# EPFL-VILAB/MultiMAE

Hardware: AMD Instinct MI355X
Metric: pre-train images/sec (whole node), ViT-B RGB+D+S 224^2 98-vis-tok (higher is better)
Workload: dtype bf16 (fp32_output_adapters: fp16 storage); 1 GPU; BASELINE.json configs[2]: ViT-B, RGB+depth+semseg, 224^2, Dirichlet alpha=1.0, 98 visible tokens, 4 cross-attention decoders (dim 256, depth 2), semseg adapter (fp32_output_adapters) with fp16 STORAGE (activations / saved tensors / gradients of the adapter as IEEE half in HBM: every matmul input carries the 11-bit significand TF32 gave the reference on A100; gradients stored times a power of two f; per_gpu_batch=256, global_batch=256, parallelism=dp1

## Files before the change

include/mmae.h:

```cpp
#ifndef MMAE_H
#define MMAE_H

#include <stddef.h>
#include <stdint.h>

#ifdef __cplusplus
extern "C" {
#endif

#define MMAE_ABI_VERSION 7

#define MMAE_F32  0
#define MMAE_BF16 1
#define MMAE_F32X3 2
#define MMAE_F32F16 3
#define MMAE_MXFP8 4

#define MMAE_F16 5

#define MMAE_EINVAL   (-1)
#define MMAE_ELAUNCH  (-2)
#define MMAE_ESUPPORT (-3)

int mmae_abi_version(void);
int mmae_struct_size(int which);
const char* mmae_last_error(void);

#define MMAE_EPI_NONE  0
#define MMAE_EPI_GELU  1
#define MMAE_EPI_DGELU 2
#define MMAE_EPI_GELU_G 3
#define MMAE_EPI_MUL   4

typedef struct mmae_gemm_desc {
    const void* A; const void* B; void* C;
    int32_t ab_dtype;
    int32_t c_dtype;
    int32_t M, N, K;
    int32_t a_trans, b_trans;
    int64_t lda, ldb, ldc;
    int32_t batch, batch_inner;
    int64_t sA_outer, sA_inner, sB_outer, sB_inner, sC_outer, sC_inner;
    const float* bias;
    const float* resid;
    int64_t ldr;
    void* aux;
    int64_t ldaux;
    int32_t aux_dtype;
    int32_t epi;
    int32_t accumulate;
    float alpha;
    int32_t tile;
    int32_t split_k;
    void* ws;
    int64_t ws_elems;
    float* colsum_part;
    float* a_colsum;
    int32_t a_colsum_acc;
    const void* a_scale;
    const void* b_scale;
    void* q_out; void* q_scale;
    int64_t ldq;
    const float* a_amax;
    const float* ln_gamma; const float* ln_beta; void* ln_out; float* ln_mean; float* ln_rstd; float ln_eps;
} mmae_gemm_desc;

int mmae_gemm(const mmae_gemm_desc* d, void* stream);
int mmae_gemm_plan(const mmae_gemm_desc* d, int* tile, int* split_k);
int mmae_gemm_auto_splitk(int M, int N, int K, int ab_dtype);
int mmae_gemm_cu_reserve(int k);
int mmae_gemm_cu_share(int k);
int mmae_gemm_side_cus(int k);
#ifdef MMAE_EXPERIMENTS
int mmae_gemm_duo_occupancy(int tile);
#endif

int64_t mmae_mx_scale_bytes(int rows, int cols);
int mmae_mx_quant(const void* x, int x_dtype, int64_t ldx, int rows, int cols, void* q, int64_t ldq, void* scales, void* stream);
int mmae_mx_quant_t(const void* w, int w_dtype, int64_t ldw, int n, int k, void* q, int64_t ldq, void* scales, void* stream);
int mmae_mx_quant_rows_t(const void* x, int x_dtype, int64_t ldx, int M, int C, void* q, int64_t ldq, void* scales, void* stream);
int mmae_mx_wgrad(int on);
int mmae_gelu_grad_aux(int on);
int mmae_ln_fuse(int on);
int mmae_xattn_fuse(int on);
int mmae_mx_scale_clear(void* scales, int rows, int cols, void* stream);
int mmae_layernorm_fwd_mx(const float* x, const float* gamma, const float* beta, void* y_bf16, float* mean, float* rstd, int64_t R, int D,
                          float eps, void* q, void* scales, void* stream);
int mmae_attn_fwd_mx(const void* q, const void* k, const void* v, void* o, float* lse, int B, int H, int Nq, int Nk, int hd,
                     int64_t q_sb, int64_t q_sr, int64_t k_sb, int64_t k_sr, int64_t v_sb, int64_t v_sr, int64_t o_sb, int64_t o_sr,
                     float scale, void* mx_q, void* mx_scale, void* stream);
int mmae_attn_bwd_mx(const void* q, const void* k, const void* v, const void* o, const void* d_o, const float* lse, void* dq, void* dk,
                     void* dv, int B, int H, int Nq, int Nk, int hd, int64_t q_sb, int64_t q_sr, int64_t k_sb, int64_t k_sr, int64_t v_sb,
                     int64_t v_sr, int64_t o_sb, int64_t o_sr, int64_t dq_sb, int64_t dq_sr, int64_t dk_sb, int64_t dk_sr, int64_t dv_sb,
                     int64_t dv_sr, float scale, void* mx_q, void* mx_scale, void* stream);
int64_t mmae_mx_tmp_bytes(int rows, int cols);
int mmae_mx_prepare_weights(int n, const void* const* w, int w_dtype, const int32_t* n_out, const int32_t* k_in, void* const* dst, void* stream);
int mmae_probe_mx_mfma(const int32_t* a_64x8, const int32_t* b_64x8, const int32_t* scale_a_64, const int32_t* scale_b_64, int opsel_a, int opsel_b,
                       float* out_64x16, void* stream);

int mmae_gemm_timing_enable(int on);
int mmae_gemm_timing_read(double* ms3, double* flop3, int64_t* calls3);
int mmae_gemm_timing_read_bytes(double* bytes3);

typedef struct mmae_dw_problem {
    const void* dy; int64_t ldy;
    const void* x; int64_t ldx;
    float* dw; float* db;
    int32_t n_out, k_in;
} mmae_dw_problem;

typedef struct mmae_dw_group_desc {
    int32_t n, rows, ab_dtype, accumulate, split_k;
    mmae_dw_problem p[8];
    float* ws; int64_t ws_elems;
    const float* unscale;
} mmae_dw_group_desc;

int64_t mmae_gemm_dw_group_ws_elems(const mmae_dw_group_desc* d);
int mmae_gemm_dw_group(const mmae_dw_group_desc* d, void* stream);

int mmae_layernorm_fwd(const float* x, const float* gamma, const float* beta, void* y, int y_dtype,
                       float* mean, float* rstd, int64_t R, int D, float eps, void* stream);
int mmae_layernorm_bwd_nblk(int64_t R);
int mmae_layernorm_bwd(const void* dy, int dy_dtype, const float* x, const float* gamma,
                       const float* mean, const float* rstd, const float* dx_in, float* dx_out,
                       void* dx_act, int dx_act_dtype, float* part, int64_t R, int D, void* stream);
int mmae_colsum_partials(const float* part, float* out, int nrows, int ncols, int accumulate, void* stream);

int64_t mmae_colsum_ws_elems(int64_t M, int N);
int mmae_colsum(const void* dy, int dtype, int64_t M, int N, int64_t ld, float* out, int accumulate,
                float* ws, void* stream);
int mmae_colsum_scatter(const void* dy, int dtype, int64_t M, int N, int64_t ld, int seg_w, const void* dsts_host,
                        int nseg, int accumulate, float* ws, void* stream);

#define MMAE_COLSUM_MAX_JOBS 8
typedef struct mmae_colsum_job {
    const void* src; int32_t dtype; int32_t cols; int64_t rows; int64_t ld;
    int32_t seg_w; int32_t nseg; float* dst[8];
    const float* unscale;
} mmae_colsum_job;
int64_t mmae_colsum_batch_ws_elems(const mmae_colsum_job* jobs, int n);
int mmae_colsum_batch(const mmae_colsum_job* jobs, int n, int accumulate, float* ws, int64_t ws_elems, void* stream);

int mmae_softmax_fwd(const float* S, int64_t lds_, void* P, int p_dtype, int64_t ldp, int64_t rows, int n,
                     float scale, void* stream);
int mmae_softmax_bwd(const void* P, int p_dtype, int64_t ldp, const float* dP, int64_t lddp, void* dS,
                     int64_t ldds, int64_t rows, int n, float scale, void* stream);

int mmae_xattn_fwd_fused(const void* qn, const void* cn, const void* wq, const float* bq, const void* wkv, const float* bkv, void* q, void* kv,
                         void* out, float* lse, int B, int H, int Nq, int Nk, int D, float scale, void* stream);
int mmae_attn_fwd(const void* q, const void* k, const void* v, void* o, float* lse, int B, int H, int Nq, int Nk, int hd,
                  int64_t q_sb, int64_t q_sr, int64_t k_sb, int64_t k_sr, int64_t v_sb, int64_t v_sr, int64_t o_sb,
                  int64_t o_sr, float scale, void* stream);
int mmae_attn_bwd(const void* q, const void* k, const void* v, const void* o, const void* d_o, const float* lse, void* dq,
                  void* dk, void* dv, int B, int H, int Nq, int Nk, int hd, int64_t q_sb, int64_t q_sr, int64_t k_sb,
                  int64_t k_sr, int64_t v_sb, int64_t v_sr, int64_t o_sb, int64_t o_sr, int64_t dq_sb, int64_t dq_sr,
                  int64_t dk_sb, int64_t dk_sr, int64_t dv_sb, int64_t dv_sr, float scale, void* stream);
int mmae_attn_fwd_f32x3(const void* q, const void* k, const void* v, void* o, float* lse, int B, int H, int Nq, int Nk, int hd,
                  int64_t q_sb, int64_t q_sr, int64_t k_sb, int64_t k_sr, int64_t v_sb, int64_t v_sr, int64_t o_sb,
                  int64_t o_sr, float scale, void* stream);
int mmae_attn_bwd_f32x3(const void* q, const void* k, const void* v, const void* o, const void* d_o, const float* lse, void* dq,
                  void* dk, void* dv, int B, int H, int Nq, int Nk, int hd, int64_t q_sb, int64_t q_sr, int64_t k_sb,
                  int64_t k_sr, int64_t v_sb, int64_t v_sr, int64_t o_sb, int64_t o_sr, int64_t dq_sb, int64_t dq_sr,
                  int64_t dk_sb, int64_t dk_sr, int64_t dv_sb, int64_t dv_sr, float scale, void* stream);
int mmae_attn_fwd_f32f16(const void* q, const void* k, const void* v, void* o, float* lse, int B, int H, int Nq, int Nk, int hd,
                  int64_t q_sb, int64_t q_sr, int64_t k_sb, int64_t k_sr, int64_t v_sb, int64_t v_sr, int64_t o_sb,
// ... 310 lines not shown
```

multimae_amd/_lib.py:

```python
from __future__ import annotations

import ctypes
import os
import re
from typing import Dict, List, Tuple

_PKG = os.path.dirname(os.path.abspath(__file__))
HEADER = os.path.join(os.path.dirname(_PKG), 'include', 'mmae.h')
LIB_PATH = os.environ.get('MMAE_LIB') or os.path.join(_PKG, 'libmmae_hip.so')

F32, BF16, F32X3, F32F16 = 0, 1, 2, 3
MXFP8 = 4
F16 = 5
U16, I32 = 6, 7
EPI_NONE, EPI_GELU, EPI_DGELU, EPI_GELU_G, EPI_MUL = 0, 1, 2, 3, 4


class GemmDesc(ctypes.Structure):
    _fields_ = [
        ('A', ctypes.c_void_p), ('B', ctypes.c_void_p), ('C', ctypes.c_void_p),
        ('ab_dtype', ctypes.c_int32), ('c_dtype', ctypes.c_int32),
        ('M', ctypes.c_int32), ('N', ctypes.c_int32), ('K', ctypes.c_int32),
        ('a_trans', ctypes.c_int32), ('b_trans', ctypes.c_int32),
        ('lda', ctypes.c_int64), ('ldb', ctypes.c_int64), ('ldc', ctypes.c_int64),
# ... 71 lines not shown


class OptGroupsDesc(ctypes.Structure):
    _fields_ = [('p', _P), ('g', _P), ('m', _P), ('v', _P), ('n', _L), ('shadow', _P), ('shadow_dtype', _I),
                ('beta1', _F), ('beta2', _F), ('eps', _F), ('clip_grad', _F), ('skip_grad', _F), ('grad_prescale', _F),
                ('loss_dev', _P), ('state', _P), ('istate', _P), ('ws', _P), ('found_inf_dev', _P), ('grad_scale_dev', _P),
                ('group_map', _P), ('n_groups', _I), ('hyper', _P), ('hyper_dev', _P)]


OPT_MAX_GROUPS = 256


class PatchSrc(ctypes.Structure):
    _fields_ = [
        ('data', ctypes.c_void_p), ('emb', ctypes.c_void_p),
        ('kind', ctypes.c_int32), ('C', ctypes.c_int32), ('H', ctypes.c_int32), ('W', ctypes.c_int32),
        ('ph', ctypes.c_int32), ('pw', ctypes.c_int32), ('k_off', ctypes.c_int32), ('n_cls', ctypes.c_int32),
    ]


_SCALARS = {
    'int': ctypes.c_int, 'int32_t': ctypes.c_int32, 'int64_t': ctypes.c_int64, 'float': ctypes.c_float,
    'size_t': ctypes.c_size_t,
}
_RET = {'int': ctypes.c_int, 'int64_t': ctypes.c_int64, 'const char*': ctypes.c_char_p}


def _parse_header(path: str) -> Dict[str, Tuple[object, List[object]]]:
    src = open(path).read()
    if not os.environ.get('MMAE_EXPERIMENTS'):
        src = re.sub(r'#ifdef\s+MMAE_EXPERIMENTS.*?#endif', ' ', src, flags=re.S)
    src = re.sub(r'/\*.*?\*/', ' ', src, flags=re.S)
    src = re.sub(r'//[^\n]*', ' ', src)
    src = re.sub(r'typedef\s+struct\s+\w+\s*\{.*?\}\s*\w+\s*;', ' ', src, flags=re.S)
    protos = {}
    for m in re.finditer(r'(const\s+char\s*\*|int64_t|int)\s+(mmae_\w+)\s*\(([^)]*)\)\s*;', src):
        ret = re.sub(r'\s+', ' ', m.group(1)).replace(' *', '*')
        name, args = m.group(2), m.group(3).strip()
        argtypes = []
        if args and args != 'void':
            for a in args.split(','):
                a = a.strip()
                if '*' in a:
                    argtypes.append(ctypes.c_void_p)
                else:
                    ty = a.split()[-2] if len(a.split()) >= 2 else a
                    argtypes.append(_SCALARS[ty])
        protos[name] = (_RET[ret], argtypes)
    return protos


_PROTOS = _parse_header(HEADER) if os.path.exists(HEADER) else {}
_lib = None


def declared_symbols() -> List[str]:
    return sorted(_PROTOS)


def load() -> ctypes.CDLL:
    global _lib
    if _lib is not None:
        return _lib
    if not os.path.exists(LIB_PATH):
        raise RuntimeError(
            f'{LIB_PATH} not found: the MI355X kernel library is not built. '
            'Run `python -c "import __graft_entry__ as g; g.build()"` (or `make -C multimae_amd/csrc`). '
            'multimae_amd has no CPU / PyTorch fallback by design.')
    lib = ctypes.CDLL(LIB_PATH)
    for name, (ret, argtypes) in _PROTOS.items():
        fn = getattr(lib, name)
        fn.restype = ret
        fn.argtypes = argtypes
    if lib.mmae_abi_version() != 7:
        raise RuntimeError('libmmae_hip.so ABI version mismatch')
    for which, cls in enumerate((GemmDesc, BlockDesc, StackDesc, AdapterDesc, OptDesc, PatchSrc, DwGroupDesc, ColsumJob,
                                     OptGroupsDesc)):
        if lib.mmae_struct_size(which) != ctypes.sizeof(cls):
            raise RuntimeError(f'{cls.__name__}: ctypes mirror ({ctypes.sizeof(cls)} B) != library struct ({lib.mmae_struct_size(which)} B)')
    if os.environ.get('MMAE_MX_WGRAD') is not None:
        lib.mmae_mx_wgrad(int(os.environ['MMAE_MX_WGRAD'] != '0'))
    if os.environ.get('MMAE_LN_FUSE') is not None:
        lib.mmae_ln_fuse(int(os.environ['MMAE_LN_FUSE'] != '0'))
    if os.environ.get('MMAE_XATTN_FUSE') is not None:
        lib.mmae_xattn_fuse(int(os.environ['MMAE_XATTN_FUSE'] != '0'))
    if os.environ.get('MMAE_GELU_GRAD_AUX') is not None:
        lib.mmae_gelu_grad_aux(int(os.environ['MMAE_GELU_GRAD_AUX'] != '0'))
    _lib = lib
    return lib


class KernelError(RuntimeError):
    pass


def check(rc: int, what: str) -> None:
    if rc != 0:
        msg = load().mmae_last_error()
        raise KernelError(f'{what} failed (rc={rc}): {msg.decode() if msg else "?"}')
```

multimae_amd/csrc/common.h:

```cpp
#pragma once
#include <hip/hip_runtime.h>
#include <stdint.h>
#include <atomic>
#include "../../include/mmae.h"

typedef __attribute__((ext_vector_type(8))) __bf16 bf16x8;
typedef __attribute__((ext_vector_type(4))) short s16x4;
typedef __attribute__((ext_vector_type(4))) int i32x4;
typedef __attribute__((ext_vector_type(2))) int i32x2;
typedef __attribute__((ext_vector_type(16))) float f32x16;
typedef __attribute__((ext_vector_type(4))) float f32x4;
typedef __attribute__((ext_vector_type(2))) float f32x2;

#define MMAE_WAVE 64

void mmae_set_error(const char* msg);
int mmae_check_launch(const char* what);
int mmae_cu_count();
int mmae_cu_side();
int mmae_cu_avail();
int mmae_depth_standardize_int(const void* x, int x_dtype, float* y, int B, int n, int lo, int hi, float eps, hipStream_t stream);

#include <stdlib.h>
static inline int mmae_env_int(const char* name, int dflt) {
// ... 98 lines not shown
    o[2] = f16_bits_to_f32((uint16_t)((uint32_t)r[1] & 0xffffu)); o[3] = f16_bits_to_f32((uint16_t)((uint32_t)r[1] >> 16));
    return o;
}
__device__ __forceinline__ void st4(h16_t* p, f32x4 v) {
    i32x2 r;
    r[0] = (int)((uint32_t)f32_to_f16_bits(v[0]) | ((uint32_t)f32_to_f16_bits(v[1]) << 16));
    r[1] = (int)((uint32_t)f32_to_f16_bits(v[2]) | ((uint32_t)f32_to_f16_bits(v[3]) << 16));
    *reinterpret_cast<i32x2*>(p) = r;
}

__device__ __forceinline__ void gelu_cdf_exp(float x, float& cdf, float& e) {
    const float z = fabsf(x) * 0.70710678118654752f;
    const float t = __builtin_amdgcn_rcpf(1.0f + 0.3275911f * z);
    float p = 1.061405429f;
    p = p * t - 1.453152027f; p = p * t + 1.421413741f; p = p * t - 0.284496736f; p = p * t + 0.254829592f;
    e = __expf(-z * z);
    const float h = 0.5f * p * t * e;
    cdf = x < 0.f ? h : 1.0f - h;
}
__device__ __forceinline__ float gelu_erf(float x) { float c, e; gelu_cdf_exp(x, c, e); return x * c; }
__device__ __forceinline__ void gelu_both(float x, float& y, float& dy) { float c, e; gelu_cdf_exp(x, c, e); y = x * c; dy = c + x * e * 0.39894228040143268f; }
__device__ __forceinline__ float gelu_erf_grad(float x) { float c, e; gelu_cdf_exp(x, c, e); return c + x * e * 0.39894228040143268f; }

__device__ __forceinline__ void gelu_both_fast2(f32x2 x, f32x2& y, f32x2& dy) {
    f32x2 t;
    t[0] = __builtin_amdgcn_fmed3f(x[0], -4.0f, 4.0f);
    t[1] = __builtin_amdgcn_fmed3f(x[1], -4.0f, 4.0f);
    const f32x2 s = t * t;
    f32x2 q = {8.063375031e-11f, 8.063375031e-11f}, r = {9.796052989e-10f, 9.796052989e-10f};
#define MMAE_PK_STEP(acc, c) acc = __builtin_elementwise_fma(acc, s, (f32x2){c, c})
    MMAE_PK_STEP(q, -7.003438364e-09f); MMAE_PK_STEP(r, -8.218800834e-08f);
    MMAE_PK_STEP(q, 2.716148569e-07f);  MMAE_PK_STEP(r, 3.028347546e-06f);
    MMAE_PK_STEP(q, -6.294988571e-06f); MMAE_PK_STEP(r, -6.495757385e-05f);
    MMAE_PK_STEP(q, 9.890799001e-05f);  MMAE_PK_STEP(r, 9.073266031e-04f);
    MMAE_PK_STEP(q, -1.133921717e-03f); MMAE_PK_STEP(r, -8.716320413e-03f);
    MMAE_PK_STEP(q, 9.877475989e-03f);  MMAE_PK_STEP(r, 5.845610030e-02f);
    MMAE_PK_STEP(q, -6.641059427e-02f); MMAE_PK_STEP(r, -2.648265329e-01f);
    MMAE_PK_STEP(q, 3.989227094e-01f);  MMAE_PK_STEP(r, 7.976095497e-01f);
#undef MMAE_PK_STEP
    const f32x2 half = {0.5f, 0.5f};
    const f32x2 cdf = __builtin_elementwise_fma(t, q, half);
    f32x2 xm;
    xm[0] = __builtin_amdgcn_fmed3f(x[0], -4.0f, 3.402823466e38f);
    xm[1] = __builtin_amdgcn_fmed3f(x[1], -4.0f, 3.402823466e38f);
    y = __builtin_elementwise_fma(xm, cdf, x * (f32x2){0.f, 0.f});
    dy = __builtin_elementwise_fma(t, r, half);
}
__device__ __forceinline__ void gelu_both_fast4(f32x4 x, f32x4& y, f32x4& dy) {
    f32x2 ya, da, yb, db;
    gelu_both_fast2((f32x2){x[0], x[1]}, ya, da);
    gelu_both_fast2((f32x2){x[2], x[3]}, yb, db);
    y = (f32x4){ya[0], ya[1], yb[0], yb[1]};
    dy = (f32x4){da[0], da[1], db[0], db[1]};
}
__device__ __forceinline__ f32x4 gelu_grad_fast4(f32x4 x) { f32x4 y, dy; gelu_both_fast4(x, y, dy); return dy; }

__device__ __forceinline__ int mx_shared_exp(float amax) {
    const unsigned b = __float_as_uint(amax);
    const int e = (int)((b >> 23) & 0xffu) - 8 + ((b & 0x7fffffu) > 0x600000u ? 1 : 0);
    return e < 0 ? 0 : e;
}
__device__ __forceinline__ float mx_inv_scale(int e) { return __uint_as_float((unsigned)(254 - e) << 23); }
__device__ __forceinline__ float mx_clamp448(float v) { return __builtin_amdgcn_fmed3f(v, -448.0f, 448.0f); }
__device__ __forceinline__ int mx_cvt4_e4m3(float a, float b, float c, float d) {
    int r = 0;
    r = __builtin_amdgcn_cvt_pk_fp8_f32(mx_clamp448(a), mx_clamp448(b), r, false);
    r = __builtin_amdgcn_cvt_pk_fp8_f32(mx_clamp448(c), mx_clamp448(d), r, true);
    return r;
}
__device__ __forceinline__ long long mx_scale_addr(long long rows, long long r, int kb) {
    return (((long long)(kb >> 3) * rows + r) * 2 + (kb & 1)) * 4 + ((kb >> 1) & 3);
}

__device__ __forceinline__ float wave_sum(float v) {
#pragma unroll
    for (int o = 32; o > 0; o >>= 1) v += __shfl_xor(v, o, 64);
    return v;
}
__device__ __forceinline__ float wave_max(float v) {
#pragma unroll
    for (int o = 32; o > 0; o >>= 1) v = fmaxf(v, __shfl_xor(v, o, 64));
    return v;
}
__device__ __forceinline__ float join4_sum(const float* sh) { return ((sh[0] + sh[1]) + sh[2]) + sh[3]; }
__device__ __forceinline__ float join4_max(const float* sh) { return fmaxf(fmaxf(sh[0], sh[1]), fmaxf(sh[2], sh[3])); }
template <class T, class Op>
__device__ __forceinline__ T block_tree(T v, T* s, Op op) {
    s[threadIdx.x] = v;
    __syncthreads();
    for (int o = 128; o > 0; o >>= 1) {
        if ((int)threadIdx.x < o) s[threadIdx.x] = op(s[threadIdx.x], s[threadIdx.x + o]);
        __syncthreads();
    }
    return s[0];
}
__device__ __forceinline__ double block_tree_sum(double v, double* s) {
    return block_tree(v, s, [](double a, double b) { return a + b; });
}
__device__ __forceinline__ float block_tree_max(float v, float* s) {
    return block_tree(v, s, [](float a, float b) { return fmaxf(a, b); });
}

__device__ __forceinline__ float resize_tap4(float ly0, float ly1, float lx0, float lx1, float a, float b, float c, float d, bool odd) {
#pragma clang fp contract(off)
    const float bot = __builtin_fmaf(lx0, c, lx1 * d);
    if (odd) {
        const float top = __builtin_fmaf(lx1, b, lx0 * a);
        return __builtin_fmaf(ly0, top, ly1 * bot);
    }
    const float top = __builtin_fmaf(lx0, a, lx1 * b);
    return __builtin_fmaf(ly1, bot, ly0 * top);
}

static inline int64_t cdiv64(int64_t a, int64_t b) { return (a + b - 1) / b; }
```

multimae_amd/csrc/composite.hip:

```cpp
#include <math.h>
#include <stdlib.h>
#include <atomic>
#include <mutex>
#include "gemm_common.h"

namespace {

struct Ctx {
    int act_dtype, f32_gemm, grad_acc;
    float* ws_main; int64_t ws_main_elems;
    float* ws_side; int64_t ws_side_elems;
    void* mx_tmp = nullptr; int64_t mx_tmp_bytes = 0;
    const void* const* x3_w = nullptr; int x3_n = 0;
    void* x3_tmp = nullptr; int64_t x3_tmp_bytes = 0;
    const float* dy_amax = nullptr;
    bool b16() const { return act_dtype != MMAE_F32; }
    bool h16() const { return act_dtype == MMAE_F16; }
    int ab() const { return b16() ? act_dtype : f32_gemm; }
    int ab_grad() const { return b16() ? act_dtype : ((f32_gemm == MMAE_F32F16 && !dy_amax) ? MMAE_F32X3 : f32_gemm); }
    const float* amax_for(int ab) const { return ab == MMAE_F32F16 ? dy_amax : nullptr; }
    const float* unscale() const { return h16() ? dy_amax : nullptr; }
    size_t es() const { return b16() ? 2 : 4; }
};
inline bool is16(int act) { return act != MMAE_F32; }
// ... 72 lines not shown
int lin_fwd(const Ctx& c, const void* x, const void* w, const float* bias, void* out, int out_dtype, int M, int N, int K,
            const float* resid, void* aux, int epi, hipStream_t st, const void* const* mxw = nullptr, int mx_in = -1, int mx_out = -1,
            const LnSide* ln = nullptr) {
    mmae_gemm_desc g = {};
    if (ln) { g.ln_gamma = ln->g; g.ln_beta = ln->b; g.ln_out = ln->out; g.ln_mean = ln->mean; g.ln_rstd = ln->rstd; g.ln_eps = ln->eps; }
    g.A = x; g.B = w; g.C = out;
    g.ab_dtype = c.ab();
    g.c_dtype = out_dtype;
    g.M = M; g.N = N; g.K = K;
    g.lda = K; g.ldb = K; g.ldc = N;
    g.batch = g.batch_inner = 1;
    g.bias = bias; g.resid = resid; g.ldr = N;
    g.aux = aux; g.ldaux = N; g.aux_dtype = c.act_dtype;
    g.epi = epi; g.alpha = 1.0f;
    bool x3p = false;
    if (!mxw) {
        int rc3 = 0;
        const void* a3 = nullptr;
        const void* const* t3 = x3_operand(c, x, K, w, M, K, &a3, st, &rc3);
        if (rc3) return rc3;
        if (t3) { g.A = a3; g.B = t3[1]; g.K = 3 * K; g.lda = g.ldb = 3LL * K; g.ab_dtype = MMAE_BF16; x3p = true; }
    }
    if (mxw) {
        int rc = mx_in_operand(c, x, K, M, K, mx_in, mx_out, &g.A, &g.a_scale, st);
        if (rc) return rc;
        if (mx_out >= 0) { if ((rc = mx_slot(c, mx_out, M, N, &g.q_out, &g.q_scale))) return rc; g.ldq = N; }
        g.B = mxw[0]; g.b_scale = mxw[1]; g.ab_dtype = MMAE_MXFP8; g.split_k = 1;
        return mmae_gemm(&g, st);
    }
    int tile = 0, split = 1;
    int rc = mmae_gemm_plan(&g, &tile, &split);
    if (rc) return rc;
    g.tile = tile; g.split_k = split;
    if (split > 1) {
        if ((int64_t)split * M * N > c.ws_main_elems) { mmae_set_error("composite: ws_main too small"); return MMAE_EINVAL; }
        g.ws = c.ws_main; g.ws_elems = c.ws_main_elems;
    }
    return x3p ? mmae_gemm_ex(&g, st, 1, 1.0 / 3.0) : mmae_gemm(&g, st);
}

int lin_dx(const Ctx& c, const void* dy, int64_t ldy, const void* w, void* out, int out_dtype, int M, int N, int K, void* aux, int epi,
           float* colsum_part, hipStream_t st, const void* const* mxw = nullptr, int mx_in = -1, int mx_out = -1) {
    mmae_gemm_desc g = {};
    g.A = dy; g.B = w; g.C = out;
    g.ab_dtype = c.ab_grad(); g.a_amax = c.amax_for(g.ab_dtype);
    if (c.h16() && out_dtype == MMAE_F32) g.a_amax = c.unscale();
    g.c_dtype = out_dtype;
    g.M = M; g.N = K; g.K = N;
    g.lda = ldy; g.ldb = K; g.ldc = K;
    g.b_trans = 1;
    g.batch = g.batch_inner = 1;
    g.aux = aux; g.ldaux = K; g.aux_dtype = c.act_dtype;
    g.epi = epi; g.alpha = 1.0f;
    g.colsum_part = colsum_part;
    bool x3p = false;
    if (!mxw) {
        int rc3 = 0;
        const void* a3 = nullptr;
        const void* const* t3 = x3_operand(c, dy, ldy, w, M, N, &a3, st, &rc3);
        if (rc3) return rc3;
        if (t3) { g.A = a3; g.lda = 3LL * N; g.B = t3[2]; g.K = 3 * N; g.ab_dtype = MMAE_BF16; x3p = true; }
    }
    if (mxw) {
        int rc = mx_in_operand(c, dy, ldy, M, N, mx_in, mx_out, &g.A, &g.a_scale, st);
        if (rc) return rc;
        if (mx_out >= 0) { if ((rc = mx_slot(c, mx_out, M, K, &g.q_out, &g.q_scale))) return rc; g.ldq = K; }
        g.lda = N; g.B = mxw[2]; g.b_scale = mxw[3]; g.ldb = N; g.b_trans = 0; g.ab_dtype = MMAE_MXFP8; g.split_k = 1;
        return mmae_gemm(&g, st);
    }
    int tile = 0, split = 1;
    int rc = mmae_gemm_plan(&g, &tile, &split);
    if (rc) return rc;
    g.tile = tile; g.split_k = split;
    if (split > 1) {
        if ((int64_t)split * M * K > c.ws_main_elems) { mmae_set_error("composite: ws_main too small"); return MMAE_EINVAL; }
        g.ws = c.ws_main; g.ws_elems = c.ws_main_elems;
    }
    return x3p ? mmae_gemm_ex(&g, st, 1, 1.0 / 3.0) : mmae_gemm(&g, st);
}

std::atomic<int> g_gelu_grad_aux{1};
inline int epi_gelu(int act) { return (is16(act) && g_gelu_grad_aux.load(std::memory_order_relaxed)) ? MMAE_EPI_GELU_G : MMAE_EPI_GELU; }
inline int epi_dgelu(int act) { return (is16(act) && g_gelu_grad_aux.load(std::memory_order_relaxed)) ? MMAE_EPI_MUL : MMAE_EPI_DGELU; }

struct ColBatch {
    mmae_colsum_job j[MMAE_COLSUM_MAX_JOBS];
    int n = 0;
    int add(const Ctx& c, const void* src, int dtype, int64_t rows, int cols, int64_t ld, int seg_w, float* const* dsts, int nseg, hipStream_t st) {
        bool any = false;
        for (int i = 0; i < nseg; ++i) any = any || dsts[i];
        if (!any) return 0;
        if (n == MMAE_COLSUM_MAX_JOBS) { const int rc = flush(c, st); if (rc) return rc; }
        mmae_colsum_job& q = j[n++];
        q = mmae_colsum_job{};
        q.src = src; q.dtype = dtype; q.rows = rows; q.cols = cols; q.ld = ld; q.seg_w = seg_w; q.nseg = nseg;
        q.unscale = c.unscale();
        for (int i = 0; i < nseg; ++i) q.dst[i] = dsts[i];
        return 0;
    }
    int add3(const Ctx& c, const float* part, int rows, int seg_w, float* d0, float* d1, float* d2, hipStream_t st) {
        float* dsts[3] = {d0, d1, d2};
        return add(c, part, MMAE_F32, rows, 3 * seg_w, 3 * seg_w, seg_w, dsts, 3, st);
    }
    int add1(const Ctx& c, const void* src, int dtype, int64_t rows, int cols, int64_t ld, float* dst, hipStream_t st) {
        float* dsts[1] = {dst};
        return add(c, src, dtype, rows, cols, ld, cols, dsts, 1, st);
    }
    int flush(const Ctx& c, hipStream_t st) {
        if (n == 0) return 0;
        const int64_t need = mmae_colsum_batch_ws_elems(j, n);
        if (need > c.ws_side_elems) { mmae_set_error("composite: ws_side too small for the batched column sums"); return MMAE_EINVAL; }
        const int rc = mmae_colsum_batch(j, n, c.grad_acc, c.ws_side, c.ws_side_elems, st);
        n = 0;
        return rc;
    }
};

int lin_dw(const Ctx& c, const void* dy, int64_t ldy, const void* x, float* dw, float* db, int M, int N, int K, hipStream_t st, ColBatch* cb = nullptr) {
    if (!dw && !db) return 0;
    const int acc = c.grad_acc;
    if (c.h16() && (dw || !cb)) { mmae_set_error("composite: an fp16-storage weight gradient outside the grouped launch (widths must be multiples of 8)"); return MMAE_ESUPPORT; }
    if (dw) {
        mmae_gemm_desc g = {};
        g.A = dy; g.B = x; g.C = dw;
        g.ab_dtype = c.ab_grad(); g.a_amax = c.amax_for(g.ab_dtype);
        g.c_dtype = MMAE_F32;
        g.M = N; g.N = K; g.K = M;
        g.lda = ldy; g.ldb = K; g.ldc = K;
        g.a_trans = g.b_trans = 1;
        g.batch = g.batch_inner = 1;
        g.accumulate = acc; g.alpha = 1.0f;
        int tile = 0, split = 1;
        int rc = mmae_gemm_plan(&g, &tile, &split);
        if (rc) return rc;
        g.tile = tile; g.split_k = split;
        const bool fused_db = db && tile == 9 && g.ab_dtype == MMAE_BF16;
        const int64_t ws_used = (split > 1 ? (int64_t)split * N * K : 0) + (fused_db ? (int64_t)(split > 1 ? split : 1) * N : 0);
        if (ws_used > c.ws_side_elems) { mmae_set_error("composite: ws_side too small"); return MMAE_EINVAL; }
        if (ws_used) { g.ws = c.ws_side; g.ws_elems = c.ws_side_elems; }
        if (fused_db) { g.a_colsum = db; g.a_colsum_acc = acc; db = nullptr; }
        rc = mmae_gemm(&g, st);
        if (rc) return rc;
    }
    if (db) {
        if (cb) return cb->add1(c, dy, c.act_dtype, M, N, ldy, db, st);
        if (mmae_colsum_ws_elems(M, N) > c.ws_side_elems) { mmae_set_error("composite: ws_side too small"); return MMAE_EINVAL; }
        return mmae_colsum(dy, c.act_dtype, M, N, ldy, db, acc, c.ws_side, st);
    }
    return 0;
}

bool dw_group_enabled() {
    static const bool on = (mmae_env_int("MMAE_DW_GROUP", 1) != 0);
    return on;
}
struct DwGroup {
    mmae_dw_group_desc g;
    bool on;
    int64_t scratch = 0;
    DwGroup(const Ctx& c, int rows) : g{}, on(c.b16() && (dw_group_enabled() || c.h16())) {
        g.rows = rows; g.ab_dtype = c.act_dtype; g.accumulate = c.grad_acc; g.unscale = c.unscale();
    }
    bool add(const void* dy, int64_t ldy, const void* x, int64_t ldx, float* dw, float* db, int n_out, int k_in) {
        if (!on || (!dw && !db) || g.n >= 8 || (n_out % 8) || (k_in % 8) || (ldy % 8) || (ldx % 8)) return false;
        mmae_dw_problem& q = g.p[g.n++];
        q.dy = dy; q.ldy = ldy; q.x = x; q.ldx = ldx; q.dw = dw; q.db = db; q.n_out = n_out; q.k_in = k_in;
// ... 174 lines not shown
    b.n1_w = p[0]; b.n1_b = p[1]; b.qkv_b = p[2]; b.proj_b = p[3]; b.n2_w = p[4]; b.n2_b = p[5]; b.fc1_b = p[6]; b.fc2_b = p[7];
}
void fill_block_act(mmae_block_desc& b, const float* x0, const BlockAct& a) {
    b.x0 = x0; b.ln1 = a.ln1; b.mean1 = a.mean1; b.rstd1 = a.rstd1; b.qkv = a.qkv; b.lse = a.lse; b.ao = a.ao; b.x1 = a.x1;
    b.ln2 = a.ln2; b.mean2 = a.mean2; b.rstd2 = a.rstd2; b.hpre = a.hpre; b.hact = a.hact; b.x2 = a.x2;
}
void fill_block_tmp(mmae_block_desc& b, const BlockTmp& t) {
    b.d_hpre = t.d_hpre; b.d_ln2 = t.d_ln2; b.d_ao = t.d_ao; b.d_qkv = t.d_qkv; b.d_ln1 = t.d_ln1; b.dx1 = t.dx1; b.dx1_act = t.dx1_act;
    b.dx0 = t.dx0; b.dx0_act = t.dx0_act; b.part_h = t.part_h; b.part1 = t.part1; b.part2 = t.part2; b.dxs_act = t.dxs_act;
}
void fill_block_grads(mmae_block_desc& b, float* const* g) {
    b.g_n1_w = g[0]; b.g_n1_b = g[1]; b.g_qkv_w = g[2]; b.g_qkv_b = g[3]; b.g_proj_w = g[4]; b.g_proj_b = g[5];
    b.g_n2_w = g[6]; b.g_n2_b = g[7]; b.g_fc1_w = g[8]; b.g_fc1_b = g[9]; b.g_fc2_w = g[10]; b.g_fc2_b = g[11];
}

struct StackRun {
    int B, N, D, heads, Hd, act, f32g, grad_acc;
    const void* const* w; const float* const* p; const float* const* dp; float* const* g;
    const float* x_in; const BlockAct* acts; BlockTmp* tmps; int nset;
    float* ws_main; int64_t ws_main_elems; float* ws_side; int64_t ws_side_elems;
    const void* const* mx_w = nullptr; void* mx_tmp = nullptr; int64_t mx_tmp_bytes = 0;
    const void* const* x3_w = nullptr; int x3_n = 0; void* x3_tmp = nullptr; int64_t x3_tmp_bytes = 0;
    const float* dy_amax = nullptr;
};

int run_blocks_bwd(const StackRun& s, int lo, int hi, const float* dx_top, const void* dx_top_act, bool top_in_sets, bool first_fc2_b_done,
                   const float* const* extra, float* cs_first, float* dx_final, hipStream_t st, hipStream_t sd,
                   const float** dx_out, const void** dx_out_act) {
    const int64_t R = (int64_t)s.B * s.N;
    const float* dx = dx_top;
    const void* dx_act = dx_top_act;
    bool fc2_done = first_fc2_b_done;
    hipEvent_t side_done[MAX_SETS] = {};
    int rc;
    MMAE_REQUIRE(s.nset >= 1 && s.nset <= MAX_SETS, "stack_bwd: more temporary sets than side-stream progress marks");
    for (int l = hi - 1; l >= lo; --l) {
        BlockTmp t = s.tmps[l % s.nset];
        if (sd != st && l + s.nset < hi + (top_in_sets ? 1 : 0) && side_done[(l + s.nset - 1) % s.nset]) {
            if (hipStreamWaitEvent(st, side_done[(l + s.nset - 1) % s.nset], 0) != hipSuccess) { mmae_set_error("stack_bwd: stream wait failed"); return MMAE_ELAUNCH; }
        }
        if (extra && l < hi - 1 && extra[l]) {
            if ((rc = mmae_axpy_f32((float*)dx, extra[l], 1.0f, R * s.D, st))) return rc;
            if ((rc = cast_to_act(s.act, dx, (void*)dx_act, R * s.D, st))) return rc;
            fc2_done = false;
        }
        mmae_block_desc b = {};
        fill_block_params(b, s.B, s.N, s.D, s.heads, s.Hd, s.act, s.f32g, 0.f, s.w + 4 * l, s.p + 8 * l);
        fill_block_act(b, l == 0 ? s.x_in : s.acts[l - 1].x2, s.acts[l]);
        if (l == lo && dx_final) { t.dx0 = dx_final; }
        fill_block_tmp(b, t);
        b.dx = dx; b.dx_act = dx_act;
        float* none[12] = {};
        fill_block_grads(b, s.g ? s.g + 12 * l : none);
        b.dp1 = s.dp ? s.dp[2 * l] : nullptr; b.dp2 = s.dp ? s.dp[2 * l + 1] : nullptr;
        const bool below_clean = l > 0 && !(extra && extra[l - 1]) && !(s.dp && s.dp[2 * (l - 1) + 1]);
        b.g_cs = l > 0 ? ((below_clean && s.g) ? s.g[12 * (l - 1) + 11] : nullptr) : cs_first;
        b.grad_acc = s.grad_acc; b.fc2_b_done = fc2_done ? 1 : 0;
        b.ws_main = s.ws_main; b.ws_main_elems = s.ws_main_elems; b.ws_side = s.ws_side; b.ws_side_elems = s.ws_side_elems;
        if (s.mx_w) { b.mx_w = s.mx_w + 16 * l; b.mx_tmp = s.mx_tmp; b.mx_tmp_bytes = s.mx_tmp_bytes; }
        b.x3_w = s.x3_w; b.x3_n = s.x3_n; b.x3_tmp = s.x3_tmp; b.x3_tmp_bytes = s.x3_tmp_bytes;
        b.dy_amax = s.dy_amax;
        if ((rc = mmae_block_bwd(&b, st, sd))) return rc;
        if (sd != st) {
            hipEvent_t e = g_held_ring.next();
            if (!e || hipEventRecord(e, sd) != hipSuccess) { mmae_set_error("stack_bwd: event record failed"); return MMAE_ELAUNCH; }
            side_done[l % s.nset] = e;
        }
        fc2_done = b.g_cs != nullptr;
        dx = t.dx0;
        dx_act = is16(s.act) ? (const void*)t.dx0_act : (const void*)t.dx0;
    }
    *dx_out = dx; *dx_out_act = dx_act;
    return 0;
}

}

int mmae_decoder_build_rows(const float* ctx, const int64_t* ids_keep, const int64_t* ids_restore, const float* mask_token,
                            const float* const* task_emb_rows, const float* pos, const int32_t* task_offsets_host, int T, int q_task, int B,
                            int n_keep, int G, int D, int n_q, float* queries, float* context, void* stream);
int mmae_decoder_build_rows_ln(const float* ctx, const int64_t* ids_keep, const int64_t* ids_restore, const float* mask_token,
                               const float* const* task_emb_rows, const float* pos, const int32_t* task_offsets_host, int T, int q_task, int B,
                               int n_keep, int G, int D, int n_q, float* queries, float* context, const BuildLn* ln, int ln_dtype, void* stream);

extern "C" {

static int block_fwd_impl(const mmae_block_desc* d, void* stream, bool ln1_done, const LnSide* next);
int mmae_block_fwd(const mmae_block_desc* d, void* stream) { return block_fwd_impl(d, stream, false, nullptr); }

static int block_fwd_impl(const mmae_block_desc* d, void* stream, bool ln1_done, const LnSide* next) {
    int rc = check_desc(d);
    if (rc) return rc;
    MMAE_REQUIRE(d->x2, "block_fwd: null output");
    MMAE_REQUIRE(!(d->dp1 || d->dp2) || d->branch, "block_fwd: stochastic depth needs the branch scratch buffer");
    hipStream_t st = (hipStream_t)stream;
    const Ctx c = ctx_of(d);
    const int R = d->B * d->N, D = d->D, Hd = d->Hd, act = d->act_dtype;
    const void* const* mx = (d->mx_w && act == MMAE_BF16) ? d->mx_w : nullptr;
    static const bool mx_fuse = (mmae_env_int("MMAE_MX_FUSE", 1) != 0);
    const int pre = (mx && mx_fuse) ? 0 : -1;
    auto ln = [&](const float* x, const float* w, const float* b, void* y, float* mu, float* rs) -> int {
        if (pre < 0) return mmae_layernorm_fwd(x, w, b, y, act, mu, rs, R, D, d->eps, st);
        void *q, *s;
        const int r0 = mx_slot(c, 0, R, D, &q, &s);
        return r0 ? r0 : mmae_layernorm_fwd_mx(x, w, b, y, mu, rs, R, D, d->eps, q, s, st);
    };
    if (!ln1_done && (rc = ln(d->x0, d->n1_w, d->n1_b, d->ln1, d->mean1, d->rstd1))) return rc;
    if ((rc = lin_fwd(c, d->ln1, d->qkv_w, d->qkv_b, d->qkv, act, R, 3 * D, D, nullptr, nullptr, MMAE_EPI_NONE, st, mx, pre))) return rc;
    const bool side = !mx && !d->dp1 && !d->dp2 && ln_side_ok(c, D, D, MMAE_F32) && (Hd % 32) == 0;
    const LnSide ln2s = {d->n2_w, d->n2_b, d->ln2, d->mean2, d->rstd2, d->eps};
    if (pre >= 0) {
        void *aq, *as;
        if ((rc = mx_slot(c, 0, R, D, &aq, &as)) || (rc = attn_strides_fwd(d, st, aq, as))) return rc;
    } else if ((rc = attn_strides_fwd(d, st))) return rc;
    if (d->dp1) {
        if ((rc = lin_fwd(c, d->ao, d->proj_w, d->proj_b, d->branch, MMAE_F32, R, D, D, nullptr, nullptr, MMAE_EPI_NONE, st, mx ? mx + 4 : nullptr, pre))) return rc;
        if ((rc = mmae_rowscale_add(d->x0, d->branch, d->dp1, d->x1, R, d->N, D, st))) return rc;
    } else {
        if ((rc = lin_fwd(c, d->ao, d->proj_w, d->proj_b, d->x1, MMAE_F32, R, D, D, d->x0, nullptr, MMAE_EPI_NONE, st, mx ? mx + 4 : nullptr, pre, -1,
                          side ? &ln2s : nullptr))) return rc;
    }
    if (!side && (rc = ln(d->x1, d->n2_w, d->n2_b, d->ln2, d->mean2, d->rstd2))) return rc;
    const int hq = pre < 0 ? -1 : 1;
    if ((rc = lin_fwd(c, d->ln2, d->fc1_w, d->fc1_b, d->hact, act, R, Hd, D, nullptr, d->hpre, epi_gelu(act), st, mx ? mx + 8 : nullptr, pre, hq))) return rc;
    if (d->dp2) {
        if ((rc = lin_fwd(c, d->hact, d->fc2_w, d->fc2_b, d->branch, MMAE_F32, R, D, Hd, nullptr, nullptr, MMAE_EPI_NONE, st, mx ? mx + 12 : nullptr, hq))) return rc;
        return mmae_rowscale_add(d->x1, d->branch, d->dp2, d->x2, R, d->N, D, st);
    }
    return lin_fwd(c, d->hact, d->fc2_w, d->fc2_b, d->x2, MMAE_F32, R, D, Hd, d->x1, nullptr, MMAE_EPI_NONE, st, mx ? mx + 12 : nullptr, hq, -1,
                   (side && next) ? next : nullptr);
}

static bool block_side_ok(const mmae_block_desc& b) {
    const Ctx c = ctx_of(&b);
    return !(b.mx_w && b.act_dtype == MMAE_BF16) && !b.dp1 && !b.dp2 && ln_side_ok(c, b.D, b.D, MMAE_F32) && (b.Hd % 32) == 0;
}

std::atomic<int> g_xattn_fuse{0};
int mmae_xattn_fuse(int on) {
    const int prev = g_xattn_fuse.load(std::memory_order_relaxed);
    if (on >= 0) g_xattn_fuse.store(on ? 1 : 0, std::memory_order_relaxed);
    return prev;
}

int mmae_ln_fuse(int on) {
    const int prev = g_ln_fuse.load(std::memory_order_relaxed);
    if (on >= 0) g_ln_fuse.store(on ? 1 : 0, std::memory_order_relaxed);
    return prev;
}

int mmae_gelu_grad_aux(int on) {
    const int prev = g_gelu_grad_aux.load(std::memory_order_relaxed);
    if (on >= 0) g_gelu_grad_aux.store(on ? 1 : 0, std::memory_order_relaxed);
    return prev;
}

int mmae_mx_wgrad(int on) {
    const int prev = g_mx_wgrad.load(std::memory_order_relaxed);
    if (on >= 0) g_mx_wgrad.store(on ? 1 : 0, std::memory_order_relaxed);
    return prev;
}

int mmae_block_bwd(const mmae_block_desc* d, void* stream, void* side_stream) {
    int rc = check_desc(d);
    if (rc) return rc;
    MMAE_REQUIRE(d->dx && d->dx_act && d->dx0 && d->d_hpre && d->d_ln2 && d->d_ao && d->d_qkv && d->d_ln1 && d->dx1 && d->part1 && d->part2,
                 "block_bwd: null gradient / temporary buffer");
    const int act = d->act_dtype;
    MMAE_REQUIRE(act == MMAE_F32 || (d->dx1_act && d->dx0_act), "block_bwd: 16-bit activations need dx1_act / dx0_act");
    MMAE_REQUIRE(act != MMAE_F16 || d->dy_amax, "block_bwd: fp16 storage needs dy_amax (the scale its gradients are stored in)");
    MMAE_REQUIRE(!d->g_fc1_b || d->part_h, "block_bwd: part_h needed for the fc1 bias gradient");
    MMAE_REQUIRE(!(d->dp1 || d->dp2) || d->dxs_act, "block_bwd: stochastic depth needs the dxs_act scratch buffer");
    MMAE_REQUIRE(!(d->dp2 && d->fc2_b_done), "block_bwd: with a scaled MLP branch the fc2 bias gradient cannot come from the producer of dx");
    hipStream_t st = (hipStream_t)stream;
    hipStream_t sd = side_stream ? (hipStream_t)side_stream : st;
    const Ctx c = ctx_of(d);
    const int R = d->B * d->N, D = d->D, Hd = d->Hd, N = d->N, hd = D / d->heads;
    const int nblk = mmae_layernorm_bwd_nblk(R);
    const int hrows = (R + 31) / 32;
    const void* dm_act = d->dx_act;
    if (d->dp2) {
        if ((rc = mmae_rowscale_cast(d->dx, d->dp2, d->dxs_act, act, R, N, D, st))) return rc;
        dm_act = d->dxs_act;
    }
    float* part_h = d->g_fc1_b ? d->part_h : nullptr;
    const void* const* mx = (d->mx_w && act == MMAE_BF16) ? d->mx_w : nullptr;
    DwGroup grp(c, R);
    if (d->dp1 || d->dp2) grp.on = false;
    ColBatch cbat;
    ColBatch* const cb_defer = (d->dp1 || d->dp2) ? nullptr : &cbat;
    auto wgrad = [&](const void* dy, int64_t ldy, const void* x, int64_t ldx, float* dw, float* db, int n_out, int k_in) -> int {
        int r = 0;
        if (mx && mx_lin_dw(c, dy, ldy, x, ldx, dw, R, n_out, k_in, sd, &r)) {
            if (r || !db) return r;
            if (mmae_colsum_ws_elems(R, n_out) > c.ws_side_elems) { mmae_set_error("composite: ws_side too small"); return MMAE_EINVAL; }
            return mmae_colsum(dy, c.act_dtype, R, n_out, ldy, db, c.grad_acc, c.ws_side, sd);
        }
        if (grp.add(dy, ldy, x, ldx, dw, db, n_out, k_in)) return 0;
        return lin_dw(c, dy, ldy, x, dw, db, R, n_out, k_in, sd, cb_defer);
    };
    static const bool mx_fuse = (mmae_env_int("MMAE_MX_FUSE", 1) != 0);
    const int hq = (mx && mx_fuse) ? 1 : -1;
    if ((rc = lin_dx(c, dm_act, D, d->fc2_w, d->d_hpre, act, R, D, Hd, d->hpre, epi_dgelu(act), part_h, st, mx ? mx + 12 : nullptr, -1, hq))) return rc;
    if ((rc = fork_to(st, sd))) return rc;
    if ((rc = wgrad(dm_act, D, d->hact, Hd, d->g_fc2_w, d->fc2_b_done ? nullptr : d->g_fc2_b, D, Hd))) return rc;
    if ((rc = lin_dx(c, d->d_hpre, Hd, d->fc1_w, d->d_ln2, act, R, Hd, D, nullptr, MMAE_EPI_NONE, nullptr, st, mx ? mx + 8 : nullptr, hq))) return rc;
    if ((rc = wgrad(d->d_hpre, Hd, d->ln2, D, d->g_fc1_w, nullptr, Hd, D))) return rc;
    if (part_h && (rc = cbat.add1(c, part_h, MMAE_F32, hrows, Hd, Hd, d->g_fc1_b, sd))) return rc;
    void* dx1_act = act == MMAE_F32 ? nullptr : d->dx1_act;
    if ((rc = mmae_layernorm_bwd(d->d_ln2, act, d->x1, d->n2_w, d->mean2, d->rstd2, d->dx, d->dx1, dx1_act, act, d->part2, R, D, st))) return rc;
    const void* da_act = act == MMAE_F32 ? (const void*)d->dx1 : (const void*)d->dx1_act;
    if (d->dp1) {
        if (d->dp2 && (rc = fork_to(sd, st))) return rc;
        if ((rc = mmae_rowscale_cast(d->dx1, d->dp1, d->dxs_act, act, R, N, D, st))) return rc;
        da_act = d->dxs_act;
    }
    if ((rc = lin_dx(c, da_act, D, d->proj_w, d->d_ao, act, R, D, D, nullptr, MMAE_EPI_NONE, nullptr, st, mx ? mx + 4 : nullptr))) return rc;
    if ((rc = fork_to(st, sd))) return rc;
    if ((rc = cbat.add3(c, d->part2, nblk, D, d->g_n2_w, d->g_n2_b, d->dp1 ? nullptr : d->g_proj_b, sd))) return rc;
    if ((rc = wgrad(da_act, D, d->ao, D, d->g_proj_w, d->dp1 ? d->g_proj_b : nullptr, D, D))) return rc;
    {
        const size_t es = es_of(act);
        const char* qkv = (const char*)d->qkv;
        char* dq = (char*)d->d_qkv;
        const int64_t sb3 = (int64_t)N * 3 * D, sb1 = (int64_t)N * D;
        auto fn = act == MMAE_BF16 ? mmae_attn_bwd : (act == MMAE_F16 ? mmae_attn_bwd_f16 : mmae_attn_bwd_f32x3);
        if (act == MMAE_F32 && c.ab_grad() == MMAE_F32F16) {
            if ((rc = mmae_attn_bwd_f32f16(qkv, qkv + (size_t)D * es, qkv + (size_t)2 * D * es, d->ao, d->d_ao, d->lse, dq, dq + (size_t)D * es,
                                           dq + (size_t)2 * D * es, d->B, d->heads, N, N, hd, sb3, 3 * D, sb3, 3 * D, sb3, 3 * D, sb1, D, sb3, 3 * D,
                                           sb3, 3 * D, sb3, 3 * D, 1.0f / sqrtf((float)hd), c.dy_amax, st))) return rc;
        } else if (N > 256) {
            const int64_t nd = (int64_t)d->B * d->heads * N;
            MMAE_REQUIRE(d->ws_main && d->ws_main_elems >= nd, "block_bwd: ws_main too small for the attention delta (B * heads * N f32)");
            if ((rc = mmae_attn_bwd_tiled(qkv, qkv + (size_t)D * es, qkv + (size_t)2 * D * es, d->ao, d->d_ao, d->lse, d->ws_main, dq, dq + (size_t)D * es,
                                          dq + (size_t)2 * D * es, d->B, d->heads, N, N, hd, sb3, 3 * D, sb3, 3 * D, sb3, 3 * D, sb1, D, sb3, 3 * D, sb3, 3 * D,
                                          sb3, 3 * D, 1.0f / sqrtf((float)hd), st))) return rc;
// ... 83 lines not shown
    MMAE_REQUIRE(d->tmp && d->tmp_bytes >= mmae_stack_tmp_bytes(d) && d->act_bytes >= mmae_stack_act_bytes(d), "stack_bwd: slab too small");
    MMAE_REQUIRE(0 <= d->l_begin && d->l_begin < d->l_end && d->l_end <= d->L, "stack_bwd: bad block range");
    MMAE_REQUIRE(d->d_out && d->d_out[d->L - 1], "stack_bwd: the gradient of the last block's output is required");
    MMAE_REQUIRE(d->l_begin > 0 || d->dx, "stack_bwd: null dx");
    hipStream_t st = (hipStream_t)stream;
    hipStream_t sd = side_stream ? (hipStream_t)side_stream : st;
    const size_t es = d->act_dtype == MMAE_BF16 ? 2 : 4;
    const bool bf = d->act_dtype == MMAE_BF16;
    const int64_t RD = (int64_t)d->B * d->N * d->D;
    Carver ca(d->act);
    BlockAct acts[64];
    for (int l = 0; l < d->L; ++l) acts[l] = carve_block_act(ca, d->B, d->N, d->D, d->heads, d->Hd, es);
    Carver ct(d->tmp);
    const int nset = d->L < NSET ? d->L : NSET;
    BlockTmp tmps[NSET];
    for (int s = 0; s < nset; ++s) tmps[s] = carve_block_tmp(ct, d->B, d->N, d->D, d->Hd, es, bf, stack_has_dp(d));
    void* top_act = bf ? ct.take(RD * es) : nullptr;
    void* mx_tmp = d->mx_w ? ct.take(stack_mx_tmp_bytes(d)) : nullptr;
    if (d->l_end < d->L && (rc = fork_to(sd, st))) return rc;
    const float* dx; const void* dx_act;
    bool fc2_done = false;
    if (d->l_end == d->L) {
        dx = d->d_out[d->L - 1];
        if (bf) { if ((rc = mmae_cast_f32_to_bf16(dx, top_act, RD, st))) return rc; dx_act = top_act; } else dx_act = dx;
    } else {
        const BlockTmp& t = tmps[d->l_end % nset];
        dx = t.dx0; dx_act = bf ? (const void*)t.dx0_act : (const void*)t.dx0;
        const int le = d->l_end;
        const bool clean = !(d->d_out[le - 1]) && !(d->dp && d->dp[2 * (le - 1) + 1]);
        fc2_done = clean && d->g && d->g[12 * (le - 1) + 11];
        if (d->d_out[le - 1]) {
            if ((rc = mmae_axpy_f32((float*)dx, d->d_out[le - 1], 1.0f, RD, st))) return rc;
            if (bf && (rc = mmae_cast_f32_to_bf16(dx, (void*)dx_act, RD, st))) return rc;
        }
    }
    StackRun s = {d->B, d->N, d->D, d->heads, d->Hd, d->act_dtype, d->f32_gemm, d->grad_acc, d->w, d->p, d->dp, d->g, d->x, acts, tmps, nset,
                  d->ws_main, d->ws_main_elems, d->ws_side, d->ws_side_elems};
    if (d->mx_w) { s.mx_w = d->mx_w; s.mx_tmp = mx_tmp; s.mx_tmp_bytes = stack_mx_tmp_bytes(d); }
    const float* o; const void* oa;
    return run_blocks_bwd(s, d->l_begin, d->l_end, dx, dx_act, d->l_end < d->L, fc2_done, d->d_out, nullptr, d->l_begin == 0 ? d->dx : nullptr, st, sd, &o, &oa);
}

namespace {

struct AdapterAct {
    float *ctx_tok, *te, *queries, *context, *qmean, *qrstd, *cmean, *crstd, *lse, *x, *omean, *orstd, *x1, *pat;
    void *enc_act, *qn, *cn, *q, *kv, *xo, *on, *hpre, *hact, *h_act;
    BlockAct blocks[MAX_SETS];
    void* x3_tmp;
};
int kp_of(const mmae_adapter_desc* d) { return d->C * d->ph * d->pw; }
int64_t adapter_x3_bytes(const mmae_adapter_desc* d) {
    if (!d->x3_w || d->act_dtype != MMAE_F32) return 0;
    int wide = d->Hd > 3 * d->D ? d->Hd : 3 * d->D;
    if (d->Denc > wide) wide = d->Denc;
    if (kp_of(d) % 32 == 0 && kp_of(d) > wide) wide = kp_of(d);
    const int64_t rq = (int64_t)d->B * d->n_q, rc = (int64_t)d->B * d->NC;
    return mmae_x3_tmp_bytes(rq > rc ? rq : rc, wide);
}

AdapterAct carve_adapter_act(Carver& cv, const mmae_adapter_desc* d) {
    const size_t es = es_of(d->act_dtype);
    const int64_t Rq = (int64_t)d->B * d->n_q, Rc = (int64_t)d->B * d->NC;
    const int D = d->D;
    AdapterAct a;
    a.enc_act = (is16(d->act_dtype) && !d->enc_act) ? cv.take(Rc * d->Denc * es) : nullptr;
    a.ctx_tok = cv.takeT<float>(Rc * D); a.te = cv.takeT<float>((int64_t)d->T * D);
    a.queries = cv.takeT<float>(Rq * D); a.context = cv.takeT<float>(Rc * D);
    a.qn = cv.take(Rq * D * es); a.cn = cv.take(Rc * D * es);
    a.qmean = cv.takeT<float>(Rq); a.qrstd = cv.takeT<float>(Rq); a.cmean = cv.takeT<float>(Rc); a.crstd = cv.takeT<float>(Rc);
    a.q = cv.take(Rq * D * es); a.kv = cv.take(Rc * 2 * D * es); a.xo = cv.take(Rq * D * es);
    a.lse = cv.takeT<float>((int64_t)d->B * d->heads * d->n_q);
    a.x = cv.takeT<float>(Rq * D); a.on = cv.take(Rq * D * es); a.omean = cv.takeT<float>(Rq); a.orstd = cv.takeT<float>(Rq);
    a.hpre = cv.take(Rq * d->Hd * es); a.hact = cv.take(Rq * d->Hd * es); a.x1 = cv.takeT<float>(Rq * D);
    for (int l = 0; l < d->depth; ++l) a.blocks[l] = carve_block_act(cv, d->B, d->n_q, D, d->heads, d->Hd, es);
    a.h_act = is16(d->act_dtype) ? cv.take(Rq * D * es) : nullptr;
    a.pat = d->pat ? d->pat : cv.takeT<float>(Rq * kp_of(d));
    a.x3_tmp = adapter_x3_bytes(d) ? cv.take(adapter_x3_bytes(d)) : nullptr;
    return a;
}

struct AdapterTmp {
    void *d_pat, *dh_act, *d_hpre, *d_on, *dx_act, *d_xo, *d_q, *d_kv, *d_qn, *d_cn, *d_ctx_act;
    float *dh, *part_h, *dx, *part_o, *d_queries, *part_q, *d_context, *part_c, *d_ctx, *part_b;
    BlockTmp blocks[MAX_SETS];
    void* x3_tmp;
};
int64_t ldpat_of(const mmae_adapter_desc* d) { return (kp_of(d) + 7) / 8 * 8; }

AdapterTmp carve_adapter_tmp(Carver& cv, const mmae_adapter_desc* d) {
    const size_t es = es_of(d->act_dtype);
    const bool bf = is16(d->act_dtype);
    const int64_t Rq = (int64_t)d->B * d->n_q, Rc = (int64_t)d->B * d->NC;
    const int D = d->D;
    AdapterTmp t;
    t.d_pat = cv.take(Rq * ldpat_of(d) * es);
    t.dh_act = cv.take(Rq * D * es);
    t.dh = bf ? cv.takeT<float>(Rq * D) : nullptr;
    for (int l = 0; l < d->depth; ++l) t.blocks[l] = carve_block_tmp(cv, d->B, d->n_q, D, d->Hd, es, bf, false);
    t.part_h = cv.takeT<float>((Rq + 31) / 32 * d->Hd);
    t.d_hpre = cv.take(Rq * d->Hd * es); t.d_on = cv.take(Rq * D * es);
    t.dx = cv.takeT<float>(Rq * D); t.dx_act = bf ? cv.take(Rq * D * es) : nullptr;
    t.part_o = cv.takeT<float>((int64_t)mmae_layernorm_bwd_nblk(Rq) * 3 * D);
    t.d_xo = cv.take(Rq * D * es); t.d_q = cv.take(Rq * D * es); t.d_kv = cv.take(Rc * 2 * D * es);
    t.d_qn = cv.take(Rq * D * es); t.d_cn = cv.take(Rc * D * es);
    t.d_queries = cv.takeT<float>(Rq * D); t.part_q = cv.takeT<float>((int64_t)mmae_layernorm_bwd_nblk(Rq) * 3 * D);
    t.d_context = cv.takeT<float>(Rc * D); t.part_c = cv.takeT<float>((int64_t)mmae_layernorm_bwd_nblk(Rc) * 3 * D);
    t.d_ctx = cv.takeT<float>(Rc * D); t.part_b = cv.takeT<float>((int64_t)mmae_decoder_build_bwd_nblk(d->B) * (d->T + 1) * D);
    t.d_ctx_act = bf ? cv.take(Rc * D * es) : nullptr;
    t.x3_tmp = adapter_x3_bytes(d) ? cv.take(adapter_x3_bytes(d)) : nullptr;
    return t;
}

int check_adapter(const mmae_adapter_desc* d) {
    MMAE_REQUIRE(d, "adapter: null descriptor");
    MMAE_REQUIRE(d->B > 0 && d->NC > 0 && d->Denc > 0 && d->D > 0 && d->heads > 0 && d->Hd > 0 && d->D % d->heads == 0 && d->depth >= 0 &&
                 d->depth <= MAX_SETS && d->T >= 1 && d->T <= 7 && d->q_task >= -1 && d->q_task < d->T && d->G >= 0 && d->n_q > 0 && d->NC > d->G,
                 "adapter: bad geometry");
    MMAE_REQUIRE(d->C > 0 && d->nh > 0 && d->nw > 0 && d->ph > 0 && d->pw > 0 && d->nh * d->nw == d->n_q, "adapter: bad patch geometry");
    MMAE_REQUIRE(d->act_dtype == MMAE_BF16 || d->act_dtype == MMAE_F16 || (d->act_dtype == MMAE_F32 && (d->f32_gemm == MMAE_F32X3 || d->f32_gemm == MMAE_F32F16)),
                 "adapter: activations must be bf16, fp16 (MMAE_F16), or f32 with split-bf16 (MMAE_F32X3) / fp16-operand (MMAE_F32F16) products");
    if (d->act_dtype == MMAE_F16 && ((d->D % 32) || (d->Denc % 32) || (d->Hd % 32) || (kp_of(d) % 8))) {
        mmae_set_error("adapter: fp16 storage needs D, Denc, Hd multiples of 32 and C * ph * pw a multiple of 8"); return MMAE_ESUPPORT;
    }
    const int hd = d->D / d->heads;
    if ((hd != 32 && hd != 64) || d->n_q > 256 || d->NC > 256) { mmae_set_error("adapter: geometry outside the fused attention kernel"); return MMAE_ESUPPORT; }
    if (d->act_dtype == MMAE_F32 && mmae_attn_bwd_lds_bytes(1, d->n_q, d->NC, hd) > MMAE_LDS_BYTES) { mmae_set_error("adapter: f32 attention tiles exceed the LDS"); return MMAE_ESUPPORT; }
    if ((d->D % 8) || (d->Denc % 8) || (d->Hd % 8) || (kp_of(d) % 4)) { mmae_set_error("adapter: widths must be multiples of 8 (patch row of 4)"); return MMAE_ESUPPORT; }
    MMAE_REQUIRE(d->task_offsets_host && d->w && d->p && d->mask_token && d->task_emb && d->pos && d->enc && d->ids_keep && d->ids_restore && d->act,
                 "adapter: null pointer");
    MMAE_REQUIRE(is16(d->act_dtype) || d->enc_act == nullptr || d->enc_act == (const void*)d->enc, "adapter: enc_act must alias enc for f32 activations");
    return 0;
}

Ctx ctx_of(const mmae_adapter_desc* d, void* x3_tmp) {
    Ctx c{d->act_dtype, d->f32_gemm, d->grad_acc, d->ws_main, d->ws_main_elems, d->ws_side, d->ws_side_elems};
    if (x3_tmp) { c.x3_w = d->x3_w; c.x3_n = d->x3_n; c.x3_tmp = x3_tmp; c.x3_tmp_bytes = adapter_x3_bytes(d); }
    c.dy_amax = d->dy_amax;
    return c;
}

}

int64_t mmae_adapter_act_bytes(const mmae_adapter_desc* d) {
    if (!d || d->depth < 0 || d->depth > MAX_SETS) return 0;
    Carver cv(nullptr);
    (void)carve_adapter_act(cv, d);
    return cv.off;
}
int64_t mmae_adapter_tmp_bytes(const mmae_adapter_desc* d) {
    if (!d || d->depth < 0 || d->depth > MAX_SETS) return 0;
    Carver cv(nullptr);
    (void)carve_adapter_tmp(cv, d);
    return cv.off;
}
int64_t mmae_adapter_pat_offset(const mmae_adapter_desc* d) {
    if (!d || d->depth < 0 || d->depth > MAX_SETS) return -1;
    Carver cv(nullptr);
    AdapterAct a = carve_adapter_act(cv, d);
    return d->pat ? -1 : (int64_t)(uintptr_t)a.pat;
}

int mmae_adapter_fwd(const mmae_adapter_desc* d, void* stream) {
    int rc = check_adapter(d);
    if (rc) return rc;
    MMAE_REQUIRE(d->act_bytes >= mmae_adapter_act_bytes(d), "adapter_fwd: activation slab too small");
    hipStream_t st = (hipStream_t)stream;
    const int act = d->act_dtype, D = d->D, Hd = d->Hd, B = d->B, NC = d->NC, n_q = d->n_q, T = d->T, depth = d->depth;
    const int Rq = B * n_q, Rc = B * NC, hd = D / d->heads, KP = kp_of(d);
    Carver cv(d->act);
    AdapterAct a = carve_adapter_act(cv, d);
    const Ctx c = ctx_of(d, a.x3_tmp);
    const size_t es = c.es();
    const void* const* w = d->w; const float* const* p = d->p;
    const void *qw = w[0], *kvw = w[1], *pw = w[2], *f1w = w[3], *f2w = w[4], *ow = w[5 + 4 * depth], *pcw = w[6 + 4 * depth];
    const float *qb = p[0], *kvb = p[1], *pb = p[2], *cnw = p[3], *cnb = p[4], *qnw = p[5], *qnb = p[6], *onw = p[7], *onb = p[8], *f1b = p[9],
                *f2b = p[10], *ob = p[11 + 8 * depth], *pcb = p[12 + 8 * depth];
    const void* enc_act = act == MMAE_F32 ? (const void*)d->enc : d->enc_act;
    if (!enc_act) {
        if ((rc = cast_to_act(act, d->enc, a.enc_act, (int64_t)Rc * d->Denc, st))) return rc;
        enc_act = a.enc_act;
    }
    if ((rc = lin_fwd(c, enc_act, pcw, pcb, a.ctx_tok, MMAE_F32, Rc, D, d->Denc, nullptr, nullptr, MMAE_EPI_NONE, st))) return rc;
    if (D <= 256) {
        const BuildLn ln = {qnw, qnb, cnw, cnb, a.qn, a.cn, a.qmean, a.qrstd, a.cmean, a.crstd, d->eps};
        if ((rc = mmae_decoder_build_rows_ln(a.ctx_tok, d->ids_keep, d->ids_restore, d->mask_token, (const float* const*)d->task_emb, d->pos, d->task_offsets_host,
                                             T, d->q_task, B, NC - d->G, d->G, D, n_q, a.queries, a.context, &ln, act, st))) return rc;
    } else {
        if ((rc = mmae_decoder_build_rows(a.ctx_tok, d->ids_keep, d->ids_restore, d->mask_token, (const float* const*)d->task_emb, d->pos, d->task_offsets_host, T,
                                          d->q_task, B, NC - d->G, d->G, D, n_q, a.queries, a.context, st))) return rc;
        if ((rc = mmae_layernorm_fwd(a.queries, qnw, qnb, a.qn, act, a.qmean, a.qrstd, Rq, D, d->eps, st))) return rc;
        if ((rc = mmae_layernorm_fwd(a.context, cnw, cnb, a.cn, act, a.cmean, a.crstd, Rc, D, d->eps, st))) return rc;
    }
    const bool xfuse = g_xattn_fuse.load(std::memory_order_relaxed) != 0 && act == MMAE_BF16 && D == 256 && d->heads == 8 && NC <= 128 && !c.x3_w;
    if (xfuse) {
        if ((rc = mmae_xattn_fwd_fused(a.qn, a.cn, qw, qb, kvw, kvb, a.q, a.kv, a.xo, a.lse, B, d->heads, n_q, NC, D, 1.0f / sqrtf((float)hd), st))) return rc;
    } else {
    if ((rc = lin_fwd(c, a.qn, qw, qb, a.q, act, Rq, D, D, nullptr, nullptr, MMAE_EPI_NONE, st))) return rc;
    if ((rc = lin_fwd(c, a.cn, kvw, kvb, a.kv, act, Rc, 2 * D, D, nullptr, nullptr, MMAE_EPI_NONE, st))) return rc;
    {
        auto fn = act == MMAE_BF16 ? mmae_attn_fwd : (act == MMAE_F16 ? mmae_attn_fwd_f16 : (d->f32_gemm == MMAE_F32F16 ? mmae_attn_fwd_f32f16 : mmae_attn_fwd_f32x3));
        const char* kv = (const char*)a.kv;
        if ((rc = fn(a.q, kv, kv + (size_t)D * es, a.xo, a.lse, B, d->heads, n_q, NC, hd, (int64_t)n_q * D, D, (int64_t)NC * 2 * D, 2 * D,
                     (int64_t)NC * 2 * D, 2 * D, (int64_t)n_q * D, D, 1.0f / sqrtf((float)hd), st))) return rc;
    }
    }
    const bool side = ln_side_ok(c, D, D, MMAE_F32) && (Hd % 32) == 0;
    const LnSide ons = {onw, onb, a.on, a.omean, a.orstd, d->eps};
    if ((rc = lin_fwd(c, a.xo, pw, pb, a.x, MMAE_F32, Rq, D, D, nullptr, nullptr, MMAE_EPI_NONE, st, nullptr, -1, -1, side ? &ons : nullptr))) return rc;
    if (!side && (rc = mmae_layernorm_fwd(a.x, onw, onb, a.on, act, a.omean, a.orstd, Rq, D, d->eps, st))) return rc;
    if ((rc = lin_fwd(c, a.on, f1w, f1b, a.hact, act, Rq, Hd, D, nullptr, a.hpre, epi_gelu(act), st))) return rc;
    auto after = [&](int l, LnSide* s) -> bool {
        if (!side) return false;
        if (l < depth) {
            const float* const* pl = p + 11 + 8 * l;
            *s = LnSide{pl[0], pl[1], a.blocks[l].ln1, a.blocks[l].mean1, a.blocks[l].rstd1, d->eps};
            return true;
        }
        if (!is16(act)) return false;
        *s = LnSide{nullptr, nullptr, a.h_act, nullptr, nullptr, 0.f};
        return true;
    };
    LnSide nx;
    bool have = after(0, &nx);
    if ((rc = lin_fwd(c, a.hact, f2w, f2b, a.x1, MMAE_F32, Rq, D, Hd, a.x, nullptr, MMAE_EPI_NONE, st, nullptr, -1, -1, have ? &nx : nullptr))) return rc;
    const float* h = a.x1;
    bool h_act_done = have && depth == 0;
    for (int l = 0; l < depth; ++l) {
        mmae_block_desc b = {};
        fill_block_params(b, B, n_q, D, d->heads, Hd, act, d->f32_gemm, d->eps, w + 5 + 4 * l, p + 11 + 8 * l);
        fill_block_act(b, h, a.blocks[l]);
        b.ws_main = d->ws_main; b.ws_main_elems = d->ws_main_elems;
        b.x3_w = c.x3_w; b.x3_n = c.x3_n; b.x3_tmp = c.x3_tmp; b.x3_tmp_bytes = c.x3_tmp_bytes;
        const bool ln1_done = have;
        LnSide nl;
        have = block_side_ok(b) && after(l + 1, &nl);
        if ((rc = block_fwd_impl(&b, st, ln1_done, have ? &nl : nullptr))) return rc;
        h = a.blocks[l].x2;
        if (l == depth - 1) h_act_done = have;
    }
    const void* h_act = h;
    if (is16(act)) { if (!h_act_done && (rc = cast_to_act(act, h, a.h_act, (int64_t)Rq * D, st))) return rc; h_act = a.h_act; }
    if ((rc = lin_fwd(c, h_act, ow, ob, a.pat, MMAE_F32, Rq, KP, D, nullptr, nullptr, MMAE_EPI_NONE, st))) return rc;
    if (d->img) return mmae_unpatchify(a.pat, d->img, B, d->C, d->nh, d->nw, d->ph, d->pw, st);
    return 0;
}

int mmae_adapter_bwd(const mmae_adapter_desc* d, void* stream, void* side_stream) {
    int rc = check_adapter(d);
    if (rc) return rc;
    MMAE_REQUIRE(d->tmp && d->tmp_bytes >= mmae_adapter_tmp_bytes(d) && d->act_bytes >= mmae_adapter_act_bytes(d), "adapter_bwd: slab too small");
    MMAE_REQUIRE((d->d_img != nullptr) != (d->d_pat != nullptr), "adapter_bwd: exactly one of d_img / d_pat");
    MMAE_REQUIRE(d->g && d->d_enc, "adapter_bwd: null gradient destination table / d_enc");
    hipStream_t st = (hipStream_t)stream;
    hipStream_t sd = side_stream ? (hipStream_t)side_stream : st;
    const int act = d->act_dtype, D = d->D, Hd = d->Hd, B = d->B, NC = d->NC, n_q = d->n_q, T = d->T, depth = d->depth;
    const int Rq = B * n_q, Rc = B * NC, hd = D / d->heads, KP = kp_of(d);
    const bool bf = is16(act);
    MMAE_REQUIRE(act != MMAE_F16 || (d->d_pat && d->dy_amax), "adapter_bwd: fp16 storage takes the loss gradient as fp16 patch rows (d_pat) in the units of dy_amax");
    Carver ca(d->act);
    AdapterAct a = carve_adapter_act(ca, d);
    Carver ct(d->tmp);
    AdapterTmp t = carve_adapter_tmp(ct, d);
    const Ctx c = ctx_of(d, t.x3_tmp);
    const size_t es = c.es();
    const void* const* w = d->w; const float* const* p = d->p;
    const void *qw = w[0], *kvw = w[1], *pw = w[2], *f1w = w[3], *f2w = w[4], *ow = w[5 + 4 * depth], *pcw = w[6 + 4 * depth];
    const float *cnw = p[3], *qnw = p[5], *onw = p[7];
    float* const* g = d->g;
    float* g_mask = g[0];
    float* const* g_temb = g + 1;
    float* const* gb = g + 1 + T;
    float* const* gblk = gb + 16;
    float* const* gtail = gblk + 12 * depth;
    const void* enc_act = act == MMAE_F32 ? (const void*)d->enc : (d->enc_act ? d->enc_act : a.enc_act);
    const void* h_act = depth > 0 ? (bf ? a.h_act : (void*)a.blocks[depth - 1].x2) : (bf ? a.h_act : (void*)a.x1);

    const void* d_pat = d->d_pat; int64_t ldp = d->ld_pat;
    if (!d_pat) {
        ldp = ldpat_of(d);
        if (ldp != KP && hipMemsetAsync(t.d_pat, 0, (size_t)Rq * ldp * es, st) != hipSuccess) { mmae_set_error("adapter_bwd: memset failed"); return MMAE_ELAUNCH; }
        if ((rc = mmae_patchify(d->d_img, t.d_pat, act, ldp, B, d->C, d->nh, d->nw, d->ph, d->pw, st))) return rc;
        d_pat = t.d_pat;
    }
    MMAE_REQUIRE(ldp >= KP && ldp % 4 == 0, "adapter_bwd: bad ld_pat");
    DwGroup grp_q(c, Rq), grp_c(c, Rc);
    ColBatch cbat;
    if ((rc = fork_to(st, sd))) return rc;
    if (!grp_q.add(d_pat, ldp, h_act, D, gtail[0], gtail[1], KP, D) && (rc = lin_dw(c, d_pat, ldp, h_act, gtail[0], gtail[1], Rq, KP, D, sd, &cbat))) return rc;
    if ((rc = lin_dx(c, d_pat, ldp, ow, t.dh_act, act, Rq, KP, D, nullptr, MMAE_EPI_NONE, nullptr, st))) return rc;
    const float* dh = (const float*)t.dh_act;
    if (bf) { if ((rc = cast_from_act(act, t.dh_act, t.dh, (int64_t)Rq * D, st))) return rc; dh = t.dh; }
    const void* dh_act = t.dh_act;
    bool fc2_done = false;
    if (depth > 0) {
        StackRun s = {B, n_q, D, d->heads, Hd, act, d->f32_gemm, d->grad_acc, w + 5, p + 11, nullptr, gblk, a.x1, a.blocks, t.blocks, depth,
                      d->ws_main, d->ws_main_elems, d->ws_side, d->ws_side_elems};
        s.x3_w = c.x3_w; s.x3_n = c.x3_n; s.x3_tmp = c.x3_tmp; s.x3_tmp_bytes = c.x3_tmp_bytes;
        s.dy_amax = c.dy_amax;
        const float* o; const void* oa;
        if ((rc = run_blocks_bwd(s, 0, depth, dh, dh_act, false, false, nullptr, gb[15], nullptr, st, sd, &o, &oa))) return rc;
        dh = o; dh_act = oa;
        fc2_done = gb[15] != nullptr;
    }
    if ((rc = lin_dx(c, dh_act, D, f2w, t.d_hpre, act, Rq, D, Hd, a.hpre, epi_dgelu(act), gb[13] ? t.part_h : nullptr, st))) return rc;
    if ((rc = fork_to(st, sd))) return rc;
    if (!grp_q.add(dh_act, D, a.hact, Hd, gb[14], fc2_done ? nullptr : gb[15], D, Hd) &&
        (rc = lin_dw(c, dh_act, D, a.hact, gb[14], fc2_done ? nullptr : gb[15], Rq, D, Hd, sd, &cbat))) return rc;
    if ((rc = lin_dx(c, t.d_hpre, Hd, f1w, t.d_on, act, Rq, Hd, D, nullptr, MMAE_EPI_NONE, nullptr, st))) return rc;
    if (!grp_q.add(t.d_hpre, Hd, a.on, D, gb[12], nullptr, Hd, D) && (rc = lin_dw(c, t.d_hpre, Hd, a.on, gb[12], nullptr, Rq, Hd, D, sd))) return rc;
    if (gb[13] && (rc = cbat.add1(c, t.part_h, MMAE_F32, (Rq + 31) / 32, Hd, Hd, gb[13], sd))) return rc;
    if ((rc = mmae_layernorm_bwd(t.d_on, act, a.x, onw, a.omean, a.orstd, dh, t.dx, bf ? t.dx_act : nullptr, act, t.part_o, Rq, D, st))) return rc;
    const void* dx_act = bf ? (const void*)t.dx_act : (const void*)t.dx;
    if ((rc = lin_dx(c, dx_act, D, pw, t.d_xo, act, Rq, D, D, nullptr, MMAE_EPI_NONE, nullptr, st))) return rc;
    if ((rc = fork_to(st, sd))) return rc;
    if ((rc = cbat.add3(c, t.part_o, mmae_layernorm_bwd_nblk(Rq), D, gb[10], gb[11], gb[5], sd))) return rc;
    if (!grp_q.add(dx_act, D, a.xo, D, gb[4], nullptr, D, D) && (rc = lin_dw(c, dx_act, D, a.xo, gb[4], nullptr, Rq, D, D, sd))) return rc;
    {
        auto fn = act == MMAE_BF16 ? mmae_attn_bwd : (act == MMAE_F16 ? mmae_attn_bwd_f16 : mmae_attn_bwd_f32x3);
        const char* kv = (const char*)a.kv; char* dkv = (char*)t.d_kv;
        if (!bf && c.ab_grad() == MMAE_F32F16) {
            if ((rc = mmae_attn_bwd_f32f16(a.q, kv, kv + (size_t)D * es, a.xo, t.d_xo, a.lse, t.d_q, dkv, dkv + (size_t)D * es, B, d->heads, n_q, NC, hd,
                                           (int64_t)n_q * D, D, (int64_t)NC * 2 * D, 2 * D, (int64_t)NC * 2 * D, 2 * D, (int64_t)n_q * D, D, (int64_t)n_q * D, D,
                                           (int64_t)NC * 2 * D, 2 * D, (int64_t)NC * 2 * D, 2 * D, 1.0f / sqrtf((float)hd), c.dy_amax, st))) return rc;
        } else
        if ((rc = fn(a.q, kv, kv + (size_t)D * es, a.xo, t.d_xo, a.lse, t.d_q, dkv, dkv + (size_t)D * es, B, d->heads, n_q, NC, hd,
                     (int64_t)n_q * D, D, (int64_t)NC * 2 * D, 2 * D, (int64_t)NC * 2 * D, 2 * D, (int64_t)n_q * D, D, (int64_t)n_q * D, D,
                     (int64_t)NC * 2 * D, 2 * D, (int64_t)NC * 2 * D, 2 * D, 1.0f / sqrtf((float)hd), st))) return rc;
    }
    if ((rc = lin_dx(c, t.d_q, D, qw, t.d_qn, act, Rq, D, D, nullptr, MMAE_EPI_NONE, nullptr, st))) return rc;
    if ((rc = lin_dx(c, t.d_kv, 2 * D, kvw, t.d_cn, act, Rc, 2 * D, D, nullptr, MMAE_EPI_NONE, nullptr, st))) return rc;
    if ((rc = fork_to(st, sd))) return rc;
    if (!grp_q.add(t.d_q, D, a.qn, D, gb[0], gb[1], D, D) && (rc = lin_dw(c, t.d_q, D, a.qn, gb[0], gb[1], Rq, D, D, sd, &cbat))) return rc;
    if (!grp_c.add(t.d_kv, 2 * D, a.cn, D, gb[2], gb[3], 2 * D, D) && (rc = lin_dw(c, t.d_kv, 2 * D, a.cn, gb[2], gb[3], Rc, 2 * D, D, sd, &cbat))) return rc;
    if ((rc = mmae_layernorm_bwd(t.d_qn, act, a.queries, qnw, a.qmean, a.qrstd, nullptr, t.d_queries, nullptr, MMAE_F32, t.part_q, Rq, D, st))) return rc;
    if ((rc = mmae_layernorm_bwd(t.d_cn, act, a.context, cnw, a.cmean, a.crstd, nullptr, t.d_context, nullptr, MMAE_F32, t.part_c, Rc, D, st))) return rc;
    if ((rc = mmae_decoder_build_bwd(t.d_queries, t.d_context, d->ids_keep, d->ids_restore, d->task_offsets_host, T, d->q_task, B, NC - d->G, d->G, D,
                                     n_q, t.d_ctx, t.part_b, st))) return rc;
    const void* d_ctx_act = t.d_ctx;
    if (bf) { if ((rc = cast_to_act(act, t.d_ctx, t.d_ctx_act, (int64_t)Rc * D, st))) return rc; d_ctx_act = t.d_ctx_act; }
    if ((rc = fork_to(st, sd))) return rc;
    if ((rc = cbat.add3(c, t.part_q, mmae_layernorm_bwd_nblk(Rq), D, gb[8], gb[9], nullptr, sd))) return rc;
    if ((rc = cbat.add3(c, t.part_c, mmae_layernorm_bwd_nblk(Rc), D, gb[6], gb[7], nullptr, sd))) return rc;
    {
        float* dst[8];
        for (int i = 0; i < T; ++i) dst[i] = g_temb[i];
        dst[T] = g_mask;
        if ((rc = cbat.add(c, t.part_b, MMAE_F32, mmae_decoder_build_bwd_nblk(B), (T + 1) * D, (T + 1) * D, D, dst, T + 1, sd))) return rc;
    }
    if (!grp_c.add(d_ctx_act, D, enc_act, d->Denc, gtail[2], gtail[3], D, d->Denc) &&
        (rc = lin_dw(c, d_ctx_act, D, enc_act, gtail[2], gtail[3], Rc, D, d->Denc, sd, &cbat))) return rc;
    if ((rc = grp_q.flush(c, sd))) return rc;
    if ((rc = grp_c.flush(c, sd))) return rc;
    if ((rc = cbat.flush(c, sd))) return rc;
    return lin_dx(c, d_ctx_act, D, pcw, d->d_enc, MMAE_F32, Rc, D, d->Denc, nullptr, MMAE_EPI_NONE, nullptr, st);
}

}
```

multimae_amd/csrc/rowops.hip:

```cpp
#include <stdlib.h>
#include <mutex>
#include <type_traits>
#include "common.h"

namespace {

template <int NV, typename YT, bool MXQ = false>
__global__ void __launch_bounds__(256) ln_fwd_kernel(const float* __restrict__ x, const float* __restrict__ gamma,
                                                     const float* __restrict__ beta, YT* __restrict__ y,
                                                     float* __restrict__ mean, float* __restrict__ rstd,
                                                     long long R, int D, float eps, unsigned char* __restrict__ qy = nullptr,
                                                     unsigned char* __restrict__ sc = nullptr) {
    const int lane = threadIdx.x & 63;
    const long long row = (long long)blockIdx.x * 4 + (threadIdx.x >> 6);
    if (row >= R) return;
    const float* xr = x + row * D;
    f32x4 v[NV];
    float s = 0.f;
#pragma unroll
    for (int i = 0; i < NV; ++i) {
        const int c = (lane + 64 * i) * 4;
        if (c < D) { v[i] = ld4(xr + c); s += (v[i][0] + v[i][1]) + (v[i][2] + v[i][3]); }
        else { v[i] = f32x4{0.f, 0.f, 0.f, 0.f}; }
    }
    const float mu = wave_sum(s) / (float)D;
    float q = 0.f;
#pragma unroll
    for (int i = 0; i < NV; ++i) {
        const int c = (lane + 64 * i) * 4;
        if (c < D) {
#pragma unroll
            for (int j = 0; j < 4; ++j) { const float d = v[i][j] - mu; q += d * d; }
        }
    }
    const float var = wave_sum(q) / (float)D;
    const float rs = 1.0f / sqrtf(var + eps);
    if (lane == 0) { mean[row] = mu; rstd[row] = rs; }
    YT* yr = y + row * D;
#pragma unroll
    for (int i = 0; i < NV; ++i) {
        const int c = (lane + 64 * i) * 4;
        if (c < D) {
            const f32x4 g = ld4(gamma + c), b = ld4(beta + c);
            f32x4 o;
#pragma unroll
            for (int j = 0; j < 4; ++j) o[j] = (v[i][j] - mu) * rs * g[j] + b[j];
            st4(yr + c, o);
            if (MXQ) {
                float w[4];
#pragma unroll
                for (int j = 0; j < 4; ++j) w[j] = bf16_bits_to_f32(f32_to_bf16_bits(o[j]));
                float am = fmaxf(fmaxf(fabsf(w[0]), fabsf(w[1])), fmaxf(fabsf(w[2]), fabsf(w[3])));
                am = fmaxf(am, __shfl_xor(am, 1, 64)); am = fmaxf(am, __shfl_xor(am, 2, 64)); am = fmaxf(am, __shfl_xor(am, 4, 64));
                const int e = mx_shared_exp(am);
                const float inv = mx_inv_scale(e);
                *reinterpret_cast<int*>(qy + row * D + c) = mx_cvt4_e4m3(w[0] * inv, w[1] * inv, w[2] * inv, w[3] * inv);
                if ((lane & 7) == 0) sc[mx_scale_addr(R, row, c >> 5)] = (unsigned char)e;
            }
        }
    }
}

template <int NV, typename DT, typename AT>
__global__ void __launch_bounds__(256) ln_bwd_kernel(const DT* __restrict__ dy, const float* __restrict__ x,
                                                     const float* __restrict__ gamma, const float* __restrict__ mean,
                                                     const float* __restrict__ rstd, const float* __restrict__ dx_in,
                                                     float* __restrict__ dx_out, AT* __restrict__ dx_act,
                                                     float* __restrict__ part, long long R, int D, int part_rows) {
    __shared__ float red[2][3][NV * 256];
    const int lane = threadIdx.x & 63, w = threadIdx.x >> 6;
    f32x4 g[NV], dg[NV], db[NV], dxs[NV];
#pragma unroll
    for (int i = 0; i < NV; ++i) {
        const int c = (lane + 64 * i) * 4;
        g[i] = (c < D) ? ld4(gamma + c) : f32x4{0.f, 0.f, 0.f, 0.f};
        dg[i] = f32x4{0.f, 0.f, 0.f, 0.f};
        db[i] = f32x4{0.f, 0.f, 0.f, 0.f};
        dxs[i] = f32x4{0.f, 0.f, 0.f, 0.f};
    }
    const long long step = (long long)gridDim.x * 4;
    long long row = (long long)blockIdx.x * 4 + w;
    f32x4 nd[NV], nx[NV], na[NV];
    float nmu = 0.f, nrs = 0.f;
    auto fetch = [&](long long r) {
        nmu = mean[r]; nrs = rstd[r];
#pragma unroll
        for (int i = 0; i < NV; ++i) {
            const int c = (lane + 64 * i) * 4;
            if (c < D) {
                nd[i] = ld4(dy + r * D + c);
                nx[i] = ld4(x + r * D + c);
                if (dx_in) na[i] = ld4(dx_in + r * D + c);
            }
        }
    };
    if (row < R) fetch(row);
    for (; row < R; row += step) {
        const float mu = nmu, rs = nrs;
        f32x4 d_[NV], xv_[NV], a_[NV];
#pragma unroll
        for (int i = 0; i < NV; ++i) { d_[i] = nd[i]; xv_[i] = nx[i]; a_[i] = na[i]; }
        if (row + step < R) fetch(row + step);
        f32x4 xh[NV], dh[NV];
        float s1 = 0.f, s2 = 0.f;
#pragma unroll
        for (int i = 0; i < NV; ++i) {
            const int c = (lane + 64 * i) * 4;
            if (c < D) {
                const f32x4 d = d_[i], xv = xv_[i];
#pragma unroll
                for (int j = 0; j < 4; ++j) {
                    xh[i][j] = (xv[j] - mu) * rs;
                    dh[i][j] = d[j] * g[i][j];
                    s1 += dh[i][j];
                    s2 += dh[i][j] * xh[i][j];
                    dg[i][j] += d[j] * xh[i][j];
                    db[i][j] += d[j];
                }
            } else { xh[i] = f32x4{0.f, 0.f, 0.f, 0.f}; dh[i] = f32x4{0.f, 0.f, 0.f, 0.f}; }
        }
        const float c1 = wave_sum(s1) / (float)D, c2 = wave_sum(s2) / (float)D;
#pragma unroll
        for (int i = 0; i < NV; ++i) {
            const int c = (lane + 64 * i) * 4;
            if (c < D) {
                f32x4 o;
#pragma unroll
                for (int j = 0; j < 4; ++j) o[j] = rs * (dh[i][j] - c1 - xh[i][j] * c2);
                if (dx_in) {
#pragma unroll
                    for (int j = 0; j < 4; ++j) o[j] += a_[i][j];
                }
                st4(dx_out + row * D + c, o);
                if (dx_act) st4(dx_act + row * D + c, o);
#pragma unroll
                for (int j = 0; j < 4; ++j) dxs[i][j] += o[j];
            }
        }
    }
    if (w < 2) {
#pragma unroll
        for (int i = 0; i < NV; ++i) {
            const int c = (lane + 64 * i) * 4;
            if (c < D) {
#pragma unroll
                for (int j = 0; j < 4; ++j) { red[w][0][c + j] = dg[i][j]; red[w][1][c + j] = db[i][j]; red[w][2][c + j] = dxs[i][j]; }
            }
        }
    }
    __syncthreads();
    if (w >= 2) {
#pragma unroll
        for (int i = 0; i < NV; ++i) {
            const int c = (lane + 64 * i) * 4;
            if (c < D) {
#pragma unroll
                for (int j = 0; j < 4; ++j) { red[w - 2][0][c + j] += dg[i][j]; red[w - 2][1][c + j] += db[i][j]; red[w - 2][2][c + j] += dxs[i][j]; }
            }
        }
    }
    __syncthreads();
    for (int c = threadIdx.x; c < 3 * D; c += 256) {
        const int k = c / D, cc = c % D;
        part[((long long)blockIdx.x * 3 + k) * D + cc] = red[0][k][cc] + red[1][k][cc];
    }
    for (long long r = (long long)blockIdx.x + gridDim.x; r < part_rows; r += gridDim.x)
        for (int c = threadIdx.x; c < 3 * D; c += 256) part[r * 3 * D + c] = 0.f;
}

struct ColDst { float* dst[8]; int seg_w; const float* unscale; };

__global__ void __launch_bounds__(256) colsum_partials_kernel(const float* __restrict__ part, const ColDst out, int nrows,
                                                              int ncols, int accumulate) {
    __shared__ float red[4][64];
    const int tx = threadIdx.x & 63, ty = threadIdx.x >> 6;
    const int c = blockIdx.x * 64 + tx;
    float s0 = 0.f, s1 = 0.f, s2 = 0.f, s3 = 0.f;
    if (c < ncols) {
        int r = ty;
        for (; r + 12 < nrows; r += 16) {
            s0 += part[(long long)(r + 0) * ncols + c]; s1 += part[(long long)(r + 4) * ncols + c];
            s2 += part[(long long)(r + 8) * ncols + c]; s3 += part[(long long)(r + 12) * ncols + c];
        }
        for (; r < nrows; r += 4) s0 += part[(long long)r * ncols + c];
    }
    red[ty][tx] = (s0 + s1) + (s2 + s3);
    __syncthreads();
    if (ty == 0 && c < ncols) {
        const float s = ((red[0][tx] + red[1][tx]) + (red[2][tx] + red[3][tx])) * h16_grad_unscale(out.unscale);
        const int seg = c / out.seg_w;
        float* o = out.dst[seg];
        if (o) { o += c - seg * out.seg_w; *o = accumulate ? *o + s : s; }
    }
}

__global__ void __launch_bounds__(256) splitk_reduce_kernel(const float* __restrict__ ws, float* __restrict__ C, int M, int N,
                                                            long long ldc, int splits, int accumulate) {
    const long long total4 = ((long long)M * N) >> 2;
    const long long slab = (long long)M * N;
    for (long long i = (long long)blockIdx.x * 256 + threadIdx.x; i < total4; i += (long long)gridDim.x * 256) {
        const long long e = i << 2;
        f32x4 a = {0.f, 0.f, 0.f, 0.f};
        int s = 0;
        for (; s + 4 <= splits; s += 4) {
            const f32x4 b0 = ld4(ws + (long long)s * slab + e), b1 = ld4(ws + (long long)(s + 1) * slab + e),
                        b2 = ld4(ws + (long long)(s + 2) * slab + e), b3 = ld4(ws + (long long)(s + 3) * slab + e);
#pragma unroll
            for (int j = 0; j < 4; ++j) a[j] += (b0[j] + b1[j]) + (b2[j] + b3[j]);
        }
        for (; s < splits; ++s) { const f32x4 b = ld4(ws + (long long)s * slab + e);
#pragma unroll
            for (int j = 0; j < 4; ++j) a[j] += b[j];
        }
        const int m = (int)(e / N), n = (int)(e % N);
        float* c = C + (long long)m * ldc + n;
// ... 751 lines not shown
```

multimae_amd/csrc/tokens.hip:

```cpp
#include "common.h"

namespace {

constexpr int MAX_TASKS = 8;

struct TaskTable { int off[MAX_TASKS + 1]; int T; };

__device__ __forceinline__ int task_of(const TaskTable& tt, int idx) {
    int t = 0;
#pragma unroll
    for (int i = 1; i < MAX_TASKS; ++i) if (i < tt.T && idx >= tt.off[i]) t = i;
    return t;
}

__global__ void __launch_bounds__(256) mask_sample_kernel(const long long* __restrict__ spt, const float* __restrict__ task_noise,
                                                          const float* __restrict__ all_noise, const TaskTable tt, int Ntot,
                                                          int n_keep, long long* __restrict__ mask_all,
                                                          long long* __restrict__ ids_keep, long long* __restrict__ ids_restore) {
    extern __shared__ float sm[];
    float* noise = sm;
    int* order = (int*)(sm + Ntot);
    const int b = blockIdx.x, tid = threadIdx.x;
    for (int j = tid; j < Ntot; j += 256) noise[j] = task_noise[(long long)b * Ntot + j];
    __syncthreads();
// ... 153 lines not shown
    const int b = (int)(rowg / (n_sel + G)), r = (int)(rowg % (n_sel + G));
    float* o = tok + rowg * D;
    if (r >= n_sel) {
        const float* gsrc = global_tok + (long long)(r - n_sel) * D;
        for (int c = threadIdx.x * 4; c < D; c += 1024) st4(o + c, ld4(gsrc + c));
        return;
    }
    const int idx = (int)sel[(long long)b * n_sel + r];
    const int t = task_of(tt, idx);
    const float* pr = proj + ((long long)b * n_sel + r) * D;
    const float* bi = tv.bias[t];
    const float* po = tv.pos[t] + (long long)(idx - tt.off[t]) * D;
    for (int c = threadIdx.x * 4; c < D; c += 1024) {
        const f32x4 a = ld4(pr + c), b4 = ld4(bi + c), p4 = ld4(po + c);
        f32x4 v;
#pragma unroll
        for (int j = 0; j < 4; ++j) v[j] = a[j] + b4[j] + p4[j];
        st4(o + c, v);
    }
}

template <typename PT>
__global__ void __launch_bounds__(256) tokens_assemble_bwd_kernel(const float* __restrict__ d_tok, PT* __restrict__ d_proj, const TaskTable tt,
                                                                  const long long* __restrict__ sel, float* __restrict__ part, int B,
                                                                  int n_sel, int G, int D) {
    const int c = threadIdx.x * 4;
    f32x4 acc[MAX_TASKS];
#pragma unroll
    for (int i = 0; i < MAX_TASKS; ++i) acc[i] = f32x4{0.f, 0.f, 0.f, 0.f};
    const long long n_rows = (long long)B * (n_sel + G);
    auto one = [&](long long rowg, const f32x4& v) {
        const int b = (int)(rowg / (n_sel + G)), r = (int)(rowg % (n_sel + G));
        int slot;
        if (r < n_sel) {
            st4(d_proj + ((long long)b * n_sel + r) * D + c, v);
            slot = task_of(tt, (int)sel[(long long)b * n_sel + r]);
        } else slot = tt.T + (r - n_sel);
#pragma unroll
        for (int i = 0; i < MAX_TASKS; ++i) if (i == slot) {
#pragma unroll
            for (int j = 0; j < 4; ++j) acc[i][j] += v[j];
        }
    };
    if (c < D) {
        long long rowg = blockIdx.x;
        for (; rowg + gridDim.x < n_rows; rowg += 2LL * gridDim.x) {
            const f32x4 v0 = ld4(d_tok + rowg * D + c), v1 = ld4(d_tok + (rowg + gridDim.x) * D + c);
            one(rowg, v0);
            one(rowg + gridDim.x, v1);
        }
        if (rowg < n_rows) one(rowg, ld4(d_tok + rowg * D + c));
    }
    if (c < D) {
        const int ns = tt.T + G;
#pragma unroll
        for (int i = 0; i < MAX_TASKS; ++i) if (i < ns) st4(part + ((long long)blockIdx.x * ns + i) * D + c, acc[i]);
    }
}

struct TePtrs { const float* p[MAX_TASKS]; };

template <typename YT>
__device__ __forceinline__ void build_ln_row(const f32x4 v, bool has, int c, int D, float eps, const float* __restrict__ g, const float* __restrict__ b,
                                              YT* __restrict__ yrow, float* __restrict__ mean, float* __restrict__ rstd, long long row, int lane) {
    const float s = has ? (v[0] + v[1]) + (v[2] + v[3]) : 0.f;
    const float mu = wave_sum(s) / (float)D;
    float q = 0.f;
    if (has) {
#pragma unroll
        for (int j = 0; j < 4; ++j) { const float d = v[j] - mu; q += d * d; }
    }
    const float var = wave_sum(q) / (float)D;
    const float rs = 1.0f / sqrtf(var + eps);
    if (lane == 0) { mean[row] = mu; rstd[row] = rs; }
    if (has) {
        const f32x4 g4 = ld4(g + c), b4 = ld4(b + c);
        f32x4 o;
#pragma unroll
        for (int j = 0; j < 4; ++j) o[j] = (v[j] - mu) * rs * g4[j] + b4[j];
        st4(yrow + c, o);
    }
}

template <typename YT, bool LN>
__global__ void __launch_bounds__(256) decoder_build_kernel(const float* __restrict__ ctx, const long long* __restrict__ ids_keep,
                                                            const long long* __restrict__ ids_restore, const float* __restrict__ mask_token,
                                                            const TePtrs tep, const float* __restrict__ pos, const TaskTable tt,
                                                            int q_task, int n_keep, int G, int D, int n_q, int Ntot,
                                                            float* __restrict__ queries, float* __restrict__ context, long long total_rows,
                                                            const BuildLn ln) {
    const int lpr = D <= 256 ? 64 : (D <= 512 ? 128 : 256);
    const int rows_per_b = n_q + n_keep + G;
    const long long grow = (long long)blockIdx.x * (256 / lpr) + threadIdx.x / lpr;
    if (grow >= total_rows) return;
    const int b = (int)(grow / rows_per_b), rr = (int)(grow % rows_per_b);
    const int tl = threadIdx.x % lpr, cstep = lpr * 4;
    const int NC = n_keep + G;
    if (rr < n_q) {
        const int j = rr;
        const long long rank = q_task < 0 ? (long long)n_keep : ids_restore[(long long)b * Ntot + tt.off[q_task] + j];
        const float* base = (rank < n_keep) ? ctx + ((long long)b * NC + rank) * D : mask_token;
        const float* te = q_task < 0 ? nullptr : tep.p[q_task];
        const float* pe = pos + (long long)j * D;
        float* o = queries + ((long long)b * n_q + j) * D;
        f32x4 v = {0.f, 0.f, 0.f, 0.f};
        for (int c = tl * 4; c < D; c += cstep) {
            const f32x4 a = ld4(base + c), t4 = te ? ld4(te + c) : f32x4{0.f, 0.f, 0.f, 0.f}, p4 = ld4(pe + c);
#pragma unroll
            for (int k = 0; k < 4; ++k) v[k] = a[k] + (t4[k] + p4[k]);
            st4(o + c, v);
        }
        if (LN) {
            const long long row = (long long)b * n_q + j;
            build_ln_row<YT>(v, tl * 4 < D, tl * 4, D, ln.eps, ln.qg, ln.qb, (YT*)ln.qn + row * D, ln.qmean, ln.qrstd, row, tl);
        }
    } else {
        const int r = rr - n_q;
        const float* src = ctx + ((long long)b * NC + r) * D;
        float* o = context + ((long long)b * NC + r) * D;
        f32x4 v = {0.f, 0.f, 0.f, 0.f};
        if (r >= n_keep) {
            for (int c = tl * 4; c < D; c += cstep) { v = ld4(src + c); st4(o + c, v); }
        } else {
            const int idx = (int)ids_keep[(long long)b * n_keep + r];
            const int t = task_of(tt, idx);
            const float* te = tep.p[t];
            const float* pe = pos + (long long)(idx - tt.off[t]) * D;
            for (int c = tl * 4; c < D; c += cstep) {
                const f32x4 a = ld4(src + c), t4 = te ? ld4(te + c) : f32x4{0.f, 0.f, 0.f, 0.f}, p4 = ld4(pe + c);
#pragma unroll
                for (int k = 0; k < 4; ++k) v[k] = a[k] + (t4[k] + p4[k]);
                st4(o + c, v);
            }
        }
        if (LN) {
            const long long row = (long long)b * NC + r;
            build_ln_row<YT>(v, tl * 4 < D, tl * 4, D, ln.eps, ln.cg, ln.cb, (YT*)ln.cn + row * D, ln.cmean, ln.crstd, row, tl);
        }
    }
}

__global__ void __launch_bounds__(256) decoder_build_bwd_kernel(const float* __restrict__ d_queries, const float* __restrict__ d_context,
                                                                const long long* __restrict__ ids_keep, const long long* __restrict__ ids_restore,
                                                                const TaskTable tt, int q_task, int B, int n_keep, int G, int D, int n_q,
                                                                int Ntot, float* __restrict__ d_ctx, float* __restrict__ part) {
    __shared__ f32x4 red[4][MAX_TASKS + 1][64];
    const int cg = D >> 2;
    const int phases = (cg <= 64) ? 4 : 1;
    const int ph = threadIdx.x / cg, lane = threadIdx.x % cg;
    const int c = lane * 4;
    const int NC = n_keep + G;
    const int split = gridDim.y;
    f32x4 acc[MAX_TASKS + 1];
#pragma unroll
    for (int i = 0; i <= MAX_TASKS; ++i) acc[i] = f32x4{0.f, 0.f, 0.f, 0.f};
    if (ph < phases) {
        const int stride = phases * split, first = blockIdx.y * phases + ph;
        for (int b = blockIdx.x; b < B; b += gridDim.x) {
            for (int rr = first; rr < NC + n_q; rr += stride) {
                if (rr < NC) {
                    const int r = rr;
                    f32x4 v = ld4(d_context + ((long long)b * NC + r) * D + c);
                    if (r < n_keep) {
                        const int idx = (int)ids_keep[(long long)b * n_keep + r];
                        const int t = task_of(tt, idx);
#pragma unroll
                        for (int i = 0; i < MAX_TASKS; ++i) if (i == t) {
#pragma unroll
                            for (int k = 0; k < 4; ++k) acc[i][k] += v[k];
                        }
                        if (t == q_task) {
                            const f32x4 q = ld4(d_queries + ((long long)b * n_q + (idx - tt.off[t])) * D + c);
#pragma unroll
                            for (int k = 0; k < 4; ++k) v[k] += q[k];
                        }
                    }
                    st4(d_ctx + ((long long)b * NC + r) * D + c, v);
                } else {
                    const int j = rr - NC;
                    const f32x4 q = ld4(d_queries + ((long long)b * n_q + j) * D + c);
                    const bool vis = q_task >= 0 && ids_restore[(long long)b * Ntot + tt.off[q_task] + j] < n_keep;
#pragma unroll
                    for (int i = 0; i < MAX_TASKS; ++i) if (i == q_task) {
#pragma unroll
                        for (int k = 0; k < 4; ++k) acc[i][k] += q[k];
                    }
                    if (!vis) {
#pragma unroll
                        for (int k = 0; k < 4; ++k) acc[MAX_TASKS][k] += q[k];
                    }
                }
            }
        }
    }
    const int ns = tt.T + 1;
    const long long prow = (long long)blockIdx.y * gridDim.x + blockIdx.x;
    if (phases == 1) {
        if (ph == 0) {
#pragma unroll
            for (int i = 0; i < MAX_TASKS; ++i) if (i < tt.T) st4(part + (prow * ns + i) * D + c, acc[i]);
            st4(part + (prow * ns + tt.T) * D + c, acc[MAX_TASKS]);
        }
        return;
    }
    if (ph < phases) {
#pragma unroll
        for (int i = 0; i <= MAX_TASKS; ++i) red[ph][i][lane] = acc[i];
    }
    __syncthreads();
    if (ph == 0) {
#pragma unroll
        for (int i = 0; i <= MAX_TASKS; ++i) {
            if (i < tt.T || i == MAX_TASKS) {
                f32x4 t = red[0][i][lane];
                for (int p = 1; p < phases; ++p) {
#pragma unroll
                    for (int k = 0; k < 4; ++k) t[k] += red[p][i][lane][k];
                }
                st4(part + (prow * ns + (i == MAX_TASKS ? tt.T : i)) * D + c, t);
            }
        }
    }
}

__global__ void unpatchify_kernel(const float* __restrict__ pat, float* __restrict__ img, int C, int nh, int nw, int ph, int pw,
                                  long long total) {
    const long long i = (long long)blockIdx.x * blockDim.x + threadIdx.x;
    if (i >= total) return;
    const int W = nw * pw, H = nh * ph;
    const int x = (int)(i % W); long long r = i / W;
    const int y = (int)(r % H); r /= H;
    const int c = (int)(r % C); const long long b = r / C;
    const int py = y / ph, iy = y % ph, px = x / pw, ix = x % pw;
    img[i] = pat[((b * nh + py) * nw + px) * ((long long)C * ph * pw) + ((long long)c * ph + iy) * pw + ix];
}
template <typename PT>
__global__ void patchify_kernel(const float* __restrict__ img, PT* __restrict__ pat, long long ld, int C, int nh, int nw, int ph, int pw,
                                long long total) {
    const long long o = (long long)blockIdx.x * blockDim.x + threadIdx.x;
    if (o >= total) return;
    const int KP = C * ph * pw;
    const int k = (int)(o % KP); long long r = o / KP;
    const int px = (int)(r % nw); r /= nw;
    const int py = (int)(r % nh); const long long b = r / nh;
    const int c = k / (ph * pw), iy = (k / pw) % ph, ix = k % pw;
    const int W = nw * pw, H = nh * ph;
    ActT<PT>::st(pat + (o / KP) * ld + k, img[((b * C + c) * H + py * ph + iy) * W + px * pw + ix]);
}

__global__ void __launch_bounds__(256) unpatchify4_kernel(const float* __restrict__ pat, float* __restrict__ img, int C, int nh, int nw,
                                                          int ph, int pw, long long total4) {
    const long long i = (long long)blockIdx.x * 256 + threadIdx.x;
    if (i >= total4) return;
    const int qn = pw >> 2;
    const int q = (int)(i % qn); long long r = i / qn;
    const int iy = (int)(r % ph); r /= ph;
    const int c = (int)(r % C); r /= C;
    const int px = (int)(r % nw); r /= nw;
    const int py = (int)(r % nh); const long long b = r / nh;
    const int W = nw * pw, H = nh * ph;
    st4(img + ((b * C + c) * H + py * ph + iy) * W + px * pw + q * 4, ld4(pat + i * 4));
}
template <typename PT>
__global__ void __launch_bounds__(256) patchify4_kernel(const float* __restrict__ img, PT* __restrict__ pat, long long ld, int C, int nh,
                                                        int nw, int ph, int pw, long long total4) {
    const long long i = (long long)blockIdx.x * 256 + threadIdx.x;
    if (i >= total4) return;
    const int qn = pw >> 2;
    const int q = (int)(i % qn); long long r = i / qn;
    const int iy = (int)(r % ph); r /= ph;
    const int c = (int)(r % C); r /= C;
    const long long tok = r;
    const int px = (int)(r % nw); r /= nw;
    const int py = (int)(r % nh); const long long b = r / nh;
    const int W = nw * pw, H = nh * ph;
    st4(pat + tok * ld + ((long long)c * ph + iy) * pw + q * 4, ld4(img + ((b * C + c) * H + py * ph + iy) * W + px * pw + q * 4));
}

template <typename PT, bool TO_PATCH>
__global__ void __launch_bounds__(256) patch_tile_kernel(const float* __restrict__ src, PT* __restrict__ dst, long long ld, int C, int nh,
                                                         int nw, int ph, int pw, int CB) {
    extern __shared__ __attribute__((aligned(16))) float tile[];
    const int W = nw * pw, H = nh * ph, ncb = (C + CB - 1) / CB;
    const int cb = blockIdx.x % ncb; long long r = blockIdx.x / ncb;
    const int py = (int)(r % nh); const long long b = r / nh;
    const int c0 = cb * CB, cn = (C - c0 < CB) ? C - c0 : CB;
    const int rowW4 = W >> 2, pw4 = pw >> 2;
    const int n_img4 = cn * ph * rowW4;
    if (TO_PATCH) {
        for (int e = threadIdx.x; e < n_img4; e += 256) {
            const int x4 = e % rowW4, rr = e / rowW4, iy = rr % ph, cl = rr / ph;
            *reinterpret_cast<f32x4*>(tile + (cl * ph + iy) * W + x4 * 4) = ld4(src + ((b * C + c0 + cl) * H + py * ph + iy) * W + x4 * 4);
        }
        __syncthreads();
        for (int e = threadIdx.x; e < n_img4; e += 256) {
            const int q = e % pw4; int rr = e / pw4;
            const int iy = rr % ph; rr /= ph;
            const int cl = rr % cn, px = rr / cn;
            const f32x4 v = *reinterpret_cast<const f32x4*>(tile + (cl * ph + iy) * W + px * pw + q * 4);
            st4(dst + ((b * nh + py) * nw + px) * ld + ((long long)(c0 + cl) * ph + iy) * pw + q * 4, v);
        }
    } else {
        for (int e = threadIdx.x; e < n_img4; e += 256) {
            const int q = e % pw4; int rr = e / pw4;
            const int iy = rr % ph; rr /= ph;
// ... 154 lines not shown
static int semseg_det_geometry(int B, int n_sel, int E, int n_cls, int* nsub_out, int* rows_per_out) {
    if (B <= 0 || n_sel <= 0 || E < 1 || E > 256 || n_cls < 1) return -1;
    int nsub = 256 / E;
    const long long tab = (long long)n_cls * E * 4;
    while (nsub > 1 && nsub * tab > 150 * 1024) --nsub;
    if (nsub * tab > (long long)MMAE_LDS_BYTES) return -1;
    const long long n_rows = (long long)B * n_sel;
    int grid = (int)(n_rows < 256 ? n_rows : 256);
    if (grid < 1) grid = 1;
    *nsub_out = nsub;
    *rows_per_out = (int)((n_rows + grid - 1) / grid);
    return (int)((n_rows + *rows_per_out - 1) / *rows_per_out);
}
int64_t mmae_semseg_emb_bwd_ws_elems(int B, int n_sel, int E, int n_cls) {
    int nsub, rows_per;
    const int grid = semseg_det_geometry(B, n_sel, E, n_cls, &nsub, &rows_per);
    return grid < 0 ? -1 : (int64_t)grid * n_cls * E;
}
int mmae_semseg_emb_bwd_det(const void* d_rows, int rows_dtype, int64_t ld, const int64_t* cls, const int64_t* sel, float* d_emb,
                            int B, int H, int W, int E, int ph, int pw, int n_sel, int k_off, int tok_off, int n_patches, int n_cls,
                            float* ws, int64_t ws_elems, int accumulate, void* stream) {
    MMAE_REQUIRE(d_rows && cls && sel && d_emb && ws && B > 0 && n_cls > 0 && E > 0, "semseg_emb_bwd_det: bad argument");
    int nsub, rows_per;
    const int grid = semseg_det_geometry(B, n_sel, E, n_cls, &nsub, &rows_per);
    if (grid < 0) { mmae_set_error("semseg_emb_bwd_det: embedding table exceeds LDS / E > 256 / no rows"); return MMAE_ESUPPORT; }
    MMAE_REQUIRE(ws_elems >= (int64_t)grid * n_cls * E, "semseg_emb_bwd_det: workspace too small (mmae_semseg_emb_bwd_ws_elems)");
    const long long n_rows = (long long)B * n_sel;
    const size_t lds = (size_t)nsub * n_cls * E * 4;
    hipStream_t st = (hipStream_t)stream;
    int rc;
    if (rows_dtype == MMAE_BF16)
        rc = mmae_launch_lds<semseg_emb_bwd_part_kernel<uint16_t>>(dim3(grid), dim3(256), lds, st, "semseg_emb_bwd_part", (const uint16_t*)d_rows, (long long)ld, (const long long*)cls, (const long long*)sel, ws, n_rows, rows_per, n_sel, H, W, E, ph, pw, k_off, tok_off, n_patches, n_cls, nsub);
    else if (rows_dtype == MMAE_F32)
        rc = mmae_launch_lds<semseg_emb_bwd_part_kernel<float>>(dim3(grid), dim3(256), lds, st, "semseg_emb_bwd_part", (const float*)d_rows, (long long)ld, (const long long*)cls, (const long long*)sel, ws, n_rows, rows_per, n_sel, H, W, E, ph, pw, k_off, tok_off, n_patches, n_cls, nsub);
    else { mmae_set_error("semseg_emb_bwd_det: bf16 / f32 rows"); return MMAE_ESUPPORT; }
    if (rc) return rc;
    const int n = n_cls * E;
    hipLaunchKernelGGL(semseg_emb_bwd_sum_kernel, dim3((n + 63) / 64), dim3(64), 0, st, (const float*)ws, d_emb, n, grid, accumulate);
    return mmae_check_launch("semseg_emb_bwd_sum");
}

int mmae_tokens_assemble(float* tok, const float* proj, const float* const* bias, const float* const* pos,
                         const int32_t* task_offsets_host, int T, const int64_t* sel, const float* global_tok, int B, int n_sel,
                         int G, int D, void* stream) {
    MMAE_REQUIRE(tok && proj && bias && pos && sel && (G == 0 || global_tok), "tokens_assemble: null pointer");
    MMAE_REQUIRE(D % 4 == 0 && D <= 1024 && B > 0 && n_sel > 0 && G >= 0, "tokens_assemble: bad sizes");
    TaskTable tt;
    MMAE_REQUIRE(fill_tt(tt, task_offsets_host, T) == 0, "tokens_assemble: 1 <= T <= 8");
    TaskVecs tv;
    for (int t = 0; t < MAX_TASKS; ++t) { tv.bias[t] = bias[t < T ? t : 0]; tv.pos[t] = pos[t < T ? t : 0]; }
    hipLaunchKernelGGL(tokens_assemble_kernel, dim3((unsigned)((long long)B * (n_sel + G))), dim3(256), 0, (hipStream_t)stream, tok,
                       proj, tv, tt, (const long long*)sel, global_tok, n_sel, G, D);
    return mmae_check_launch("tokens_assemble");
}

int mmae_tokens_assemble_bwd_nblk(int B) { const long long n = 4LL * B; return (int)(n < 1024 ? n : 1024); }

int mmae_tokens_assemble_bwd(const float* d_tok, void* d_proj, int proj_dtype, const int32_t* task_offsets_host, int T,
                             const int64_t* sel, float* part, int B, int n_sel, int G, int D, void* stream) {
    MMAE_REQUIRE(d_tok && d_proj && sel && part, "tokens_assemble_bwd: null pointer");
    MMAE_REQUIRE(D % 4 == 0 && D <= 1024 && T + G <= MAX_TASKS, "tokens_assemble_bwd: bad sizes");
    TaskTable tt;
    MMAE_REQUIRE(fill_tt(tt, task_offsets_host, T) == 0, "tokens_assemble_bwd: 1 <= T <= 8");
    const int nblk = mmae_tokens_assemble_bwd_nblk(B);
    hipStream_t st = (hipStream_t)stream;
    if (proj_dtype == MMAE_BF16) hipLaunchKernelGGL((tokens_assemble_bwd_kernel<uint16_t>), dim3(nblk), dim3(256), 0, st, d_tok, (uint16_t*)d_proj, tt, (const long long*)sel, part, B, n_sel, G, D);
    else hipLaunchKernelGGL((tokens_assemble_bwd_kernel<float>), dim3(nblk), dim3(256), 0, st, d_tok, (float*)d_proj, tt, (const long long*)sel, part, B, n_sel, G, D);
    return mmae_check_launch("tokens_assemble_bwd");
}

}
int mmae_decoder_build_rows_ln(const float* ctx, const int64_t* ids_keep, const int64_t* ids_restore, const float* mask_token,
                               const float* const* task_emb_rows, const float* pos, const int32_t* task_offsets_host, int T, int q_task, int B,
                               int n_keep, int G, int D, int n_q, float* queries, float* context, const BuildLn* ln, int ln_dtype, void* stream);
int mmae_decoder_build_rows(const float* ctx, const int64_t* ids_keep, const int64_t* ids_restore, const float* mask_token,
                            const float* const* task_emb_rows, const float* pos, const int32_t* task_offsets_host, int T, int q_task, int B,
                            int n_keep, int G, int D, int n_q, float* queries, float* context, void* stream) {
    return mmae_decoder_build_rows_ln(ctx, ids_keep, ids_restore, mask_token, task_emb_rows, pos, task_offsets_host, T, q_task, B, n_keep, G, D, n_q,
                                      queries, context, nullptr, MMAE_F32, stream);
}
int mmae_decoder_build_rows_ln(const float* ctx, const int64_t* ids_keep, const int64_t* ids_restore, const float* mask_token,
                               const float* const* task_emb_rows, const float* pos, const int32_t* task_offsets_host, int T, int q_task, int B,
                               int n_keep, int G, int D, int n_q, float* queries, float* context, const BuildLn* ln, int ln_dtype, void* stream) {
    MMAE_REQUIRE(ctx && ids_keep && ids_restore && mask_token && task_emb_rows && pos && queries && context, "decoder_build: null pointer");
    MMAE_REQUIRE(D % 4 == 0 && D <= 1024 && B > 0, "decoder_build: bad sizes");
    TaskTable tt;
    MMAE_REQUIRE(fill_tt(tt, task_offsets_host, T) == 0 && q_task >= -1 && q_task < T, "decoder_build: bad task table");
    MMAE_REQUIRE(n_q > 0 && (q_task < 0 || tt.off[q_task + 1] - tt.off[q_task] == n_q), "decoder_build: n_q != tokens of the query task");
    TePtrs tep = {};
    for (int t = 0; t < T; ++t) {
        MMAE_REQUIRE(((uintptr_t)task_emb_rows[t] % 16) == 0, "decoder_build: unaligned task embedding");
        tep.p[t] = task_emb_rows[t];
    }
    const int rpw = D <= 256 ? 4 : (D <= 512 ? 2 : 1);
    const long long total_rows = (long long)B * (n_q + n_keep + G);
    const dim3 grid((unsigned)((total_rows + rpw - 1) / rpw));
    hipStream_t st = (hipStream_t)stream;
    const BuildLn none = {};
#define DB_LAUNCH(YT, LN, L) hipLaunchKernelGGL((decoder_build_kernel<YT, LN>), grid, dim3(256), 0, st, ctx, (const long long*)ids_keep, \
                       (const long long*)ids_restore, mask_token, tep, pos, tt, q_task, n_keep, G, D, n_q, tt.off[T], queries, context, total_rows, L)
    if (ln) {
        MMAE_REQUIRE(D <= 256 && ln->qg && ln->qb && ln->cg && ln->cb && ln->qn && ln->cn && ln->qmean && ln->qrstd && ln->cmean && ln->crstd,
                     "decoder_build: the fused LayerNorm needs D <= 256 and every output");
        if (ln_dtype == MMAE_BF16) DB_LAUNCH(uint16_t, true, *ln);
        else if (ln_dtype == MMAE_F16) DB_LAUNCH(h16_t, true, *ln);
        else DB_LAUNCH(float, true, *ln);
    } else DB_LAUNCH(float, false, none);
#undef DB_LAUNCH
    return mmae_check_launch("decoder_build");
}
extern "C" {

int mmae_decoder_build(const float* ctx, const int64_t* ids_keep, const int64_t* ids_restore, const float* mask_token,
                       const float* task_emb, const float* pos, const int32_t* task_offsets_host, int T, int q_task, int B,
                       int n_keep, int G, int D, int n_q, float* queries, float* context, void* stream) {
    MMAE_REQUIRE(task_emb && T >= 1 && T <= MAX_TASKS, "decoder_build: null task embedding table / bad task count");
    const float* rows[MAX_TASKS];
    for (int t = 0; t < T; ++t) rows[t] = task_emb + (long long)t * D;
    return mmae_decoder_build_rows(ctx, ids_keep, ids_restore, mask_token, rows, pos, task_offsets_host, T, q_task, B, n_keep, G, D, n_q,
                                   queries, context, stream);
}

static int dbb_split(int B) { return B <= 512 ? 4 : 1; }
int mmae_decoder_build_bwd_nblk(int B) { return (B < 1024 ? B : 1024) * dbb_split(B); }

int mmae_decoder_build_bwd(const float* d_queries, const float* d_context, const int64_t* ids_keep, const int64_t* ids_restore,
                           const int32_t* task_offsets_host, int T, int q_task, int B, int n_keep, int G, int D, int n_q,
                           float* d_ctx, float* part, void* stream) {
    MMAE_REQUIRE(d_queries && d_context && ids_keep && ids_restore && d_ctx && part, "decoder_build_bwd: null pointer");
    MMAE_REQUIRE(D % 4 == 0 && D <= 1024 && B > 0, "decoder_build_bwd: bad sizes");
    TaskTable tt;
    MMAE_REQUIRE(fill_tt(tt, task_offsets_host, T) == 0 && q_task >= -1 && q_task < T, "decoder_build_bwd: bad task table");
    hipLaunchKernelGGL(decoder_build_bwd_kernel, dim3(B < 1024 ? B : 1024, dbb_split(B)), dim3(256), 0, (hipStream_t)stream, d_queries,
                       d_context, (const long long*)ids_keep, (const long long*)ids_restore, tt, q_task, B, n_keep, G, D, n_q,
                       tt.off[T], d_ctx, part);
    return mmae_check_launch("decoder_build_bwd");
}

int mmae_unpatchify(const float* patches, float* img, int B, int C, int nh, int nw, int ph, int pw, void* stream) {
    MMAE_REQUIRE(patches && img && B > 0 && C > 0, "unpatchify: bad argument");
    const long long total = (long long)B * C * nh * ph * nw * pw;
    const int cbu = (pw % 4 == 0 && pw < 16) ? patch_tile_cb(ph, nw * pw) : 0;
    if (cbu > 0 && ((uintptr_t)patches % 16 == 0) && ((uintptr_t)img % 16 == 0)) {
        const long long nblk = (long long)B * nh * ((C + cbu - 1) / cbu);
        hipLaunchKernelGGL((patch_tile_kernel<float, false>), dim3((unsigned)nblk), dim3(256), (size_t)cbu * ph * nw * pw * 4, (hipStream_t)stream,
                           patches, img, (long long)C * ph * pw, C, nh, nw, ph, pw, cbu);
        return mmae_check_launch("unpatchify");
    }
    if (pw % 4 == 0 && ((uintptr_t)patches % 16 == 0) && ((uintptr_t)img % 16 == 0))
        hipLaunchKernelGGL(unpatchify4_kernel, dim3((unsigned)cdiv64(total / 4, 256)), dim3(256), 0, (hipStream_t)stream, patches, img, C,
                           nh, nw, ph, pw, total / 4);
    else
        hipLaunchKernelGGL(unpatchify_kernel, dim3((unsigned)cdiv64(total, 256)), dim3(256), 0, (hipStream_t)stream, patches, img, C, nh, nw,
                           ph, pw, total);
    return mmae_check_launch("unpatchify");
}

int mmae_patchify(const float* img, void* patches, int patches_dtype, int64_t ld, int B, int C, int nh, int nw, int ph, int pw, void* stream) {
    MMAE_REQUIRE(patches && img && B > 0 && C > 0 && ld >= (int64_t)C * ph * pw, "patchify: bad argument");
    if (patches_dtype != MMAE_BF16 && patches_dtype != MMAE_F32) { mmae_set_error("patchify: bf16 / f32 patches"); return MMAE_ESUPPORT; }
    const long long total = (long long)B * C * nh * ph * nw * pw;
    hipStream_t st = (hipStream_t)stream;
    const int cbp = (pw % 4 == 0 && pw < 16 && ld % 4 == 0) ? patch_tile_cb(ph, nw * pw) : 0;
    if (cbp > 0 && ((uintptr_t)patches % 16 == 0) && ((uintptr_t)img % 16 == 0)) {
        const dim3 grid((unsigned)((long long)B * nh * ((C + cbp - 1) / cbp)));
        const size_t lds = (size_t)cbp * ph * nw * pw * 4;
        if (patches_dtype == MMAE_BF16) hipLaunchKernelGGL((patch_tile_kernel<uint16_t, true>), grid, dim3(256), lds, st, img, (uint16_t*)patches, (long long)ld, C, nh, nw, ph, pw, cbp);
        else hipLaunchKernelGGL((patch_tile_kernel<float, true>), grid, dim3(256), lds, st, img, (float*)patches, (long long)ld, C, nh, nw, ph, pw, cbp);
        return mmae_check_launch("patchify");
    }
    if (pw % 4 == 0 && ld % 4 == 0 && ((uintptr_t)patches % 16 == 0) && ((uintptr_t)img % 16 == 0)) {
        const dim3 grid((unsigned)cdiv64(total / 4, 256));
        if (patches_dtype == MMAE_BF16) hipLaunchKernelGGL((patchify4_kernel<uint16_t>), grid, dim3(256), 0, st, img, (uint16_t*)patches, (long long)ld, C, nh, nw, ph, pw, total / 4);
        else hipLaunchKernelGGL((patchify4_kernel<float>), grid, dim3(256), 0, st, img, (float*)patches, (long long)ld, C, nh, nw, ph, pw, total / 4);
        return mmae_check_launch("patchify");
    }
    if (patches_dtype == MMAE_BF16) hipLaunchKernelGGL((patchify_kernel<uint16_t>), dim3((unsigned)cdiv64(total, 256)), dim3(256), 0, st, img, (uint16_t*)patches, (long long)ld, C, nh, nw, ph, pw, total);
    else hipLaunchKernelGGL((patchify_kernel<float>), dim3((unsigned)cdiv64(total, 256)), dim3(256), 0, st, img, (float*)patches, (long long)ld, C, nh, nw, ph, pw, total);
    return mmae_check_launch("patchify");
}

int mmae_semseg_avg_emb_fwd(const int64_t* x, const float* class_emb, float* out, int B, int H, int W, int E, int ph, int pw, int n_cls, void* stream) {
    MMAE_REQUIRE(x && class_emb && out && B > 0 && H > 0 && W > 0 && E > 0 && ph > 0 && pw > 0 && H % ph == 0 && W % pw == 0 && n_cls > 0, "semseg_avg_emb_fwd: bad argument");
    const long long total = (long long)B * E * (H / ph) * (W / pw);
    hipLaunchKernelGGL(semseg_avg_emb_fwd_kernel, dim3((unsigned)((total + 255) / 256 < 8192 ? (total + 255) / 256 : 8192)), dim3(256), 0, (hipStream_t)stream,
                       (const long long*)x, class_emb, out, B, H, W, E, ph, pw, n_cls);
    return mmae_check_launch("semseg_avg_emb_fwd");
}
int mmae_semseg_avg_emb_bwd(const float* d_img, const int64_t* x, float* d_class_emb, int B, int H, int W, int E, int ph, int pw, int n_cls, int pad_idx,
                            void* stream) {
    MMAE_REQUIRE(d_img && x && d_class_emb && B > 0 && H > 0 && W > 0 && E > 0 && ph > 0 && pw > 0 && H % ph == 0 && W % pw == 0 && n_cls > 0, "semseg_avg_emb_bwd: bad argument");
    const long long total = (long long)B * E * (H / ph) * (W / pw);
// ... 27 lines not shown
```

multimae_amd/ops.py:

```python
from __future__ import annotations

import ctypes
import math
from typing import Optional, Sequence

import torch

from . import _lib
import contextlib

from ._lib import BF16, F16, F32, F32X3, F32F16, MXFP8, EPI_NONE, EPI_GELU, EPI_DGELU, EPI_GELU_G, EPI_MUL, AdapterDesc, BlockDesc, DwGroupDesc, GemmDesc, OptDesc, OptGroupsDesc, PatchSrc, StackDesc, check

Tensor = torch.Tensor


def _require_gpu(t: Tensor, name: str = 'tensor') -> None:
    if not t.is_cuda:
        raise RuntimeError(f'multimae_amd: {name} is on {t.device}; the engine runs on MI355X HIP kernels only '
                           '(no CPU / PyTorch fallback). Move the model and inputs to a GPU.')


def dcode(dtype: torch.dtype) -> int:
    if dtype == torch.float32:
        return F32
# ... 127 lines not shown
    check(_lib.load().mmae_mx_quant(x.data_ptr(), dcode(x.dtype), x.stride(0), rows, cols, out.q.data_ptr(), cols, out.scales.data_ptr(),
                                    _stream()), 'mmae_mx_quant')
    return out


def mx_empty(rows: int, cols: int, device) -> MxTensor:
    return MxTensor(torch.empty((rows, cols), device=device, dtype=torch.uint8),
                    torch.zeros((mx_scale_bytes(rows, cols),), device=device, dtype=torch.uint8), rows, cols)


def layernorm_fwd_mx(x: Tensor, w: Tensor, b: Tensor, eps: float):
    _require_gpu(x, 'layernorm input')
    R, D = x.shape
    y = torch.empty((R, D), device=x.device, dtype=torch.bfloat16)
    mean = torch.empty((R,), device=x.device, dtype=torch.float32)
    rstd = torch.empty_like(mean)
    q = mx_empty(R, D, x.device)
    check(_lib.load().mmae_layernorm_fwd_mx(x.data_ptr(), w.data_ptr(), b.data_ptr(), y.data_ptr(), mean.data_ptr(), rstd.data_ptr(), R, D, eps,
                                            q.q.data_ptr(), q.scales.data_ptr(), _stream()), 'mmae_layernorm_fwd_mx')
    return y, mean, rstd, q


def mx_quant_t(w: Tensor, out: Optional[MxTensor] = None) -> MxTensor:
    _require_gpu(w, 'mx_quant_t input')
    n, k = w.shape
    if out is None:
        out = MxTensor(torch.empty((k, n), device=w.device, dtype=torch.uint8),
                       torch.empty((mx_scale_bytes(k, n),), device=w.device, dtype=torch.uint8), k, n)
    check(_lib.load().mmae_mx_quant_t(w.data_ptr(), dcode(w.dtype), w.stride(0), n, k, out.q.data_ptr(), n, out.scales.data_ptr(),
                                      _stream()), 'mmae_mx_quant_t')
    return out


def mx_quant_rows_t(x: Tensor) -> MxTensor:
    _require_gpu(x, 'mx_quant_rows_t input')
    M, C = x.shape
    Mp = round_up(M, 256)
    out = MxTensor(torch.empty((C, Mp), device=x.device, dtype=torch.uint8),
                   torch.empty((mx_scale_bytes(C, Mp),), device=x.device, dtype=torch.uint8), C, Mp)
    check(_lib.load().mmae_mx_quant_rows_t(x.data_ptr(), dcode(x.dtype), x.stride(0), M, C, out.q.data_ptr(), Mp, out.scales.data_ptr(),
                                           _stream()), 'mmae_mx_quant_rows_t')
    return out


def mx_wgrad(on: Optional[bool] = None) -> bool:
    return bool(_lib.load().mmae_mx_wgrad(-1 if on is None else int(bool(on))))


def gemm_mx(a: MxTensor, b: MxTensor, C: Tensor, *, bias: Optional[Tensor] = None, resid: Optional[Tensor] = None,
            aux: Optional[Tensor] = None, epi: int = EPI_NONE, colsum_part: Optional[Tensor] = None,
            q_out: Optional[MxTensor] = None, split_k: int = 1, accumulate: bool = False) -> Tensor:
    assert a.cols == b.cols, (a.cols, b.cols)
    M, N, K = a.rows, b.rows, a.cols
    d = GemmDesc()
    d.A, d.B, d.C = a.q.data_ptr(), b.q.data_ptr(), C.data_ptr()
    d.a_scale, d.b_scale = a.scales.data_ptr(), b.scales.data_ptr()
    d.ab_dtype, d.c_dtype = MXFP8, dcode(C.dtype)
    d.M, d.N, d.K = M, N, K
    d.lda, d.ldb, d.ldc = K, K, N
    d.batch = d.batch_inner = 1
    d.bias = _p(bias)
    d.resid, d.ldr = _p(resid), N
    d.aux, d.ldaux = _p(aux), N
    d.aux_dtype = dcode(aux.dtype) if aux is not None else F32
    d.epi, d.alpha, d.split_k = epi, 1.0, split_k
    d.accumulate = int(accumulate)
    if split_k > 1:
        ws = stream_workspace(_stream(), C.device, max(_WS_ELEMS[0], split_k * M * N))
        d.ws, d.ws_elems = ws.data_ptr(), ws.numel()
    d.colsum_part = _p(colsum_part)
    if q_out is not None:
        assert q_out.rows == M and q_out.cols == N
        d.q_out, d.q_scale, d.ldq = q_out.q.data_ptr(), q_out.scales.data_ptr(), N
    check(_lib.load().mmae_gemm(ctypes.byref(d), _stream()), 'mmae_gemm(mxfp8)')
    return C


def gemm_cu_reserve(k: Optional[int] = None) -> int:
    return int(_lib.load().mmae_gemm_cu_reserve(-1 if k is None else int(k)))


def ln_fuse(on: Optional[bool] = None) -> bool:
    return bool(_lib.load().mmae_ln_fuse(-1 if on is None else int(bool(on))))


def xattn_fuse(on: Optional[bool] = None) -> bool:
    return bool(_lib.load().mmae_xattn_fuse(-1 if on is None else int(bool(on))))


def gemm_cu_share(k: Optional[int] = None) -> int:
    return int(_lib.load().mmae_gemm_cu_share(-1 if k is None else int(k)))


def gemm_side_cus(k: Optional[int] = None) -> int:
    return int(_lib.load().mmae_gemm_side_cus(-1 if k is None else int(k)))


def linear_fwd(x: Tensor, w: Tensor, bias: Optional[Tensor], out: Tensor, *, resid: Optional[Tensor] = None,
               aux: Optional[Tensor] = None, epi: int = EPI_NONE, tile: int = 0, ln: Optional[tuple] = None) -> Tensor:
    M, K = x.shape
    N = w.shape[0]
    gemm(x, w, out, M, N, K, lda=K, ldb=K, ldc=N, bias=bias, resid=resid, ldr=N, aux=aux, ldaux=N, epi=epi, tile=tile, ln=ln)
    return out


def linear_dx(dy: Tensor, w: Tensor, out: Tensor, *, aux: Optional[Tensor] = None, epi: int = EPI_NONE,
              colsum_out: Optional[Tensor] = None, colsum_part: Optional[Tensor] = None, tile: int = 0) -> Tensor:
    M, N = dy.shape
    K = w.shape[1]
    part = colsum_part
    if colsum_out is not None and part is None:
        part = torch.empty(dx_colsum_part_shape(M, K), device=dy.device, dtype=torch.float32)
    gemm(dy, w, out, M, K, N, lda=dy.stride(0), ldb=K, ldc=K, b_trans=True, aux=aux, ldaux=K, epi=epi, colsum_part=part, tile=tile)
    if colsum_out is not None:
        colsum(part, colsum_out, False)
    return out


def gemm_dw_group(problems: Sequence[tuple], accumulate: bool, split_k: int = 0, unscale: Optional[Tensor] = None) -> None:
    d = DwGroupDesc()
    ab = problems[0][0].dtype
    d.n, d.rows, d.ab_dtype, d.accumulate, d.split_k = len(problems), problems[0][0].shape[0], dcode(ab), int(accumulate), split_k
    d.unscale = _p(unscale)
    for i, (dy, x, dw, db) in enumerate(problems):
        assert ab in (torch.bfloat16, torch.float16) and dy.dtype == ab and x.dtype == ab and dw.dtype == torch.float32 and dw.is_contiguous()
        assert dy.shape[0] == d.rows and x.shape[0] == d.rows and dw.shape == (dy.shape[1], x.shape[1])
        q = d.p[i]
        q.dy, q.ldy, q.x, q.ldx, q.dw, q.db, q.n_out, q.k_in = dy.data_ptr(), dy.stride(0), x.data_ptr(), x.stride(0), dw.data_ptr(), _p(db), dy.shape[1], x.shape[1]
    lib = _lib.load()
    n_ws = lib.mmae_gemm_dw_group_ws_elems(ctypes.byref(d))
    ws = torch.empty((max(n_ws, 4),), device=problems[0][0].device, dtype=torch.float32)
    d.ws, d.ws_elems = ws.data_ptr(), ws.numel()
    check(lib.mmae_gemm_dw_group(ctypes.byref(d), _stream()), 'gemm_dw_group')


def dx_colsum_part_shape(M: int, K: int):
    return ((M + 31) // 32, K)


def linear_dw(dy: Tensor, x: Tensor, dw: Tensor, accumulate: bool, *, db: Optional[Tensor] = None, db_accumulate: bool = False,
              x_off: int = 0, ldx: Optional[int] = None, K: Optional[int] = None) -> Tensor:
    M, N = dy.shape
    K = K if K is not None else x.shape[1]
    fused = gemm(dy, x, dw, N, K, M, lda=dy.stride(0), ldb=ldx if ldx is not None else x.stride(0), ldc=K, a_trans=True, b_trans=True,
                 b_off=x_off, accumulate=accumulate, a_colsum=db, a_colsum_acc=db_accumulate)
    if db is not None and not fused:
        colsum(dy, db, db_accumulate)
    return dw


_COMPOSITE = [_os.environ.get('MMAE_COMPOSITE', '1') != '0']
_WS = {}
_WS_ELEMS = [56 << 20]


def _device_ok(t: Tensor) -> bool:
    return t.is_cuda


def set_composite_blocks(flag: bool) -> None:
    _COMPOSITE[0] = bool(flag)


def stream_workspace(stream_handle: int, device, elems: Optional[int] = None) -> Tensor:
    elems = elems or _WS_ELEMS[0]
    key = (str(device), stream_handle)
# ... 1248 lines not shown
```

Baseline: 8934 images/s.

## Fuse decoder-build backward with both LayerNorm backwards and skip saving pre-LN rows

In the adapter backward, two LayerNorm backward passes, the decoder-build backward and the cast of d_ctx to the activation dtype are replaced by one kernel. That kernel recomputes the pre-LN query and context rows from ctx, the task embeddings and pos, writes d_ctx directly in the activation dtype, and emits per-block partial sums for the LN weights and embeddings. Because the rows are recomputed, the forward build kernel no longer stores the fp32 queries and context tensors. This removes several full read/write passes and kernel launches over the decoder rows. In exchange it adds recompute work, a new partial buffer and reduction job, and somewhat different rounding order, exposed through ln_bwd_terms helpers with contraction turned off.

```diff
diff --git a/include/mmae.h b/include/mmae.h
--- a/include/mmae.h
+++ b/include/mmae.h
@@ -82,6 +82,7 @@
 int mmae_mx_wgrad(int on);
 int mmae_gelu_grad_aux(int on);
 int mmae_ln_fuse(int on);
+int mmae_build_fuse(int on);
 int mmae_xattn_fuse(int on);
 int mmae_mx_scale_clear(void* scales, int rows, int cols, void* stream);
 int mmae_layernorm_fwd_mx(const float* x, const float* gamma, const float* beta, void* y_bf16, float* mean, float* rstd, int64_t R, int D,
diff --git a/multimae_amd/_lib.py b/multimae_amd/_lib.py
--- a/multimae_amd/_lib.py
+++ b/multimae_amd/_lib.py
@@ -177,6 +177,8 @@
         lib.mmae_mx_wgrad(int(os.environ['MMAE_MX_WGRAD'] != '0'))
     if os.environ.get('MMAE_LN_FUSE') is not None:
         lib.mmae_ln_fuse(int(os.environ['MMAE_LN_FUSE'] != '0'))
+    if os.environ.get('MMAE_BUILD_FUSE') is not None:
+        lib.mmae_build_fuse(int(os.environ['MMAE_BUILD_FUSE'] != '0'))
     if os.environ.get('MMAE_XATTN_FUSE') is not None:
         lib.mmae_xattn_fuse(int(os.environ['MMAE_XATTN_FUSE'] != '0'))
     if os.environ.get('MMAE_GELU_GRAD_AUX') is not None:
diff --git a/multimae_amd/csrc/common.h b/multimae_amd/csrc/common.h
--- a/multimae_amd/csrc/common.h
+++ b/multimae_amd/csrc/common.h
@@ -204,6 +204,41 @@
     for (int o = 32; o > 0; o >>= 1) v = fmaxf(v, __shfl_xor(v, o, 64));
     return v;
 }
+__device__ __forceinline__ void ln_bwd_terms(const f32x4 d, const f32x4 xv, const f32x4 g, float mu, float rs, f32x4& xh, f32x4& dh,
+                                             float& s1, float& s2, f32x4& dg, f32x4& db) {
+#pragma clang fp contract(off)
+#pragma unroll
+    for (int j = 0; j < 4; ++j) {
+        xh[j] = (xv[j] - mu) * rs;
+        dh[j] = d[j] * g[j];
+        s1 = s1 + dh[j];
+        s2 = s2 + dh[j] * xh[j];
+        dg[j] = __builtin_fmaf(d[j], xh[j], dg[j]);
+        db[j] = db[j] + d[j];
+    }
+}
+__device__ __forceinline__ f32x4 ln_bwd_dx(const f32x4 xh, const f32x4 dh, float rs, float c1, float c2) {
+#pragma clang fp contract(off)
+    f32x4 o;
+#pragma unroll
+    for (int j = 0; j < 4; ++j) o[j] = rs * __builtin_fmaf(-c2, xh[j], dh[j] - c1);
+    return o;
+}
+__device__ __forceinline__ f32x4 ln_bwd_dx_add(const f32x4 xh, const f32x4 dh, float rs, float c1, float c2, const f32x4 a) {
+#pragma clang fp contract(off)
+    f32x4 o;
+#pragma unroll
+    for (int j = 0; j < 4; ++j) o[j] = __builtin_fmaf(rs, __builtin_fmaf(-c2, xh[j], dh[j] - c1), a[j]);
+    return o;
+}
+__device__ __forceinline__ f32x4 add4_rn(const f32x4 a, const f32x4 b) {
+#pragma clang fp contract(off)
+    f32x4 o;
+#pragma unroll
+    for (int j = 0; j < 4; ++j) o[j] = a[j] + b[j];
+    return o;
+}
+
 __device__ __forceinline__ float join4_sum(const float* sh) { return ((sh[0] + sh[1]) + sh[2]) + sh[3]; }
 __device__ __forceinline__ float join4_max(const float* sh) { return fmaxf(fmaxf(sh[0], sh[1]), fmaxf(sh[2], sh[3])); }
 template <class T, class Op>
diff --git a/multimae_amd/csrc/composite.hip b/multimae_amd/csrc/composite.hip
--- a/multimae_amd/csrc/composite.hip
+++ b/multimae_amd/csrc/composite.hip
@@ -178,6 +178,10 @@
 std::atomic<int> g_gelu_grad_aux{1};
 inline int epi_gelu(int act) { return (is16(act) && g_gelu_grad_aux.load(std::memory_order_relaxed)) ? MMAE_EPI_GELU_G : MMAE_EPI_GELU; }
 inline int epi_dgelu(int act) { return (is16(act) && g_gelu_grad_aux.load(std::memory_order_relaxed)) ? MMAE_EPI_MUL : MMAE_EPI_DGELU; }
+std::atomic<int> g_build_fuse{1};
+inline bool build_fused(int D) {
+    return D <= 256 && g_build_fuse.load(std::memory_order_relaxed) != 0 && g_ln_fuse.load(std::memory_order_relaxed) != 0;
+}
 
 struct ColBatch {
     mmae_colsum_job j[MMAE_COLSUM_MAX_JOBS];
@@ -518,6 +522,10 @@
 int mmae_decoder_build_rows_ln(const float* ctx, const int64_t* ids_keep, const int64_t* ids_restore, const float* mask_token,
                                const float* const* task_emb_rows, const float* pos, const int32_t* task_offsets_host, int T, int q_task, int B,
                                int n_keep, int G, int D, int n_q, float* queries, float* context, const BuildLn* ln, int ln_dtype, void* stream);
+int mmae_decoder_build_bwd_ln_nblk(int64_t units);
+int mmae_decoder_build_bwd_ln(const void* d_qn, const void* d_cn, int dtype, const float* ctx, const int64_t* ids_keep, const int64_t* ids_restore,
+                              const float* mask_token, const float* const* task_emb_rows, const float* pos, const int32_t* task_offsets_host, int T,
+                              int q_task, int B, int n_keep, int G, int D, int n_q, const BuildLn* ln, void* d_ctx, float* part, void* stream);
 
 extern "C" {
 
@@ -588,6 +596,12 @@
 int mmae_gelu_grad_aux(int on) {
     const int prev = g_gelu_grad_aux.load(std::memory_order_relaxed);
     if (on >= 0) g_gelu_grad_aux.store(on ? 1 : 0, std::memory_order_relaxed);
+    return prev;
+}
+
+int mmae_build_fuse(int on) {
+    const int prev = g_build_fuse.load(std::memory_order_relaxed);
+    if (on >= 0) g_build_fuse.store(on ? 1 : 0, std::memory_order_relaxed);
     return prev;
 }
 
@@ -837,7 +851,7 @@
 
 struct AdapterTmp {
     void *d_pat, *dh_act, *d_hpre, *d_on, *dx_act, *d_xo, *d_q, *d_kv, *d_qn, *d_cn, *d_ctx_act;
-    float *dh, *part_h, *dx, *part_o, *d_queries, *part_q, *d_context, *part_c, *d_ctx, *part_b;
+    float *dh, *part_h, *dx, *part_o, *d_queries, *part_q, *d_context, *part_c, *d_ctx, *part_b, *part_f;
     BlockTmp blocks[MAX_SETS];
     void* x3_tmp;
 };
@@ -863,6 +877,7 @@
     t.d_context = cv.takeT<float>(Rc * D); t.part_c = cv.takeT<float>((int64_t)mmae_layernorm_bwd_nblk(Rc) * 3 * D);
     t.d_ctx = cv.takeT<float>(Rc * D); t.part_b = cv.takeT<float>((int64_t)mmae_decoder_build_bwd_nblk(d->B) * (d->T + 1) * D);
     t.d_ctx_act = bf ? cv.take(Rc * D * es) : nullptr;
+    t.part_f = D <= 256 ? cv.takeT<float>((int64_t)mmae_decoder_build_bwd_ln_nblk(Rq + Rc) * (d->T + 5) * D) : nullptr;
     t.x3_tmp = adapter_x3_bytes(d) ? cv.take(adapter_x3_bytes(d)) : nullptr;
     return t;
 }
@@ -939,8 +954,9 @@
     if ((rc = lin_fwd(c, enc_act, pcw, pcb, a.ctx_tok, MMAE_F32, Rc, D, d->Denc, nullptr, nullptr, MMAE_EPI_NONE, st))) return rc;
     if (D <= 256) {
         const BuildLn ln = {qnw, qnb, cnw, cnb, a.qn, a.cn, a.qmean, a.qrstd, a.cmean, a.crstd, d->eps};
+        const bool save = !build_fused(D);
         if ((rc = mmae_decoder_build_rows_ln(a.ctx_tok, d->ids_keep, d->ids_restore, d->mask_token, (const float* const*)d->task_emb, d->pos, d->task_offsets_host,
-                                             T, d->q_task, B, NC - d->G, d->G, D, n_q, a.queries, a.context, &ln, act, st))) return rc;
+                                             T, d->q_task, B, NC - d->G, d->G, D, n_q, save ? a.queries : nullptr, save ? a.context : nullptr, &ln, act, st))) return rc;
     } else {
         if ((rc = mmae_decoder_build_rows(a.ctx_tok, d->ids_keep, d->ids_restore, d->mask_token, (const float* const*)d->task_emb, d->pos, d->task_offsets_host, T,
                                           d->q_task, B, NC - d->G, d->G, D, n_q, a.queries, a.context, st))) return rc;
@@ -1088,20 +1104,29 @@
     if ((rc = fork_to(st, sd))) return rc;
     if (!grp_q.add(t.d_q, D, a.qn, D, gb[0], gb[1], D, D) && (rc = lin_dw(c, t.d_q, D, a.qn, gb[0], gb[1], Rq, D, D, sd, &cbat))) return rc;
     if (!grp_c.add(t.d_kv, 2 * D, a.cn, D, gb[2], gb[3], 2 * D, D) && (rc = lin_dw(c, t.d_kv, 2 * D, a.cn, gb[2], gb[3], Rc, 2 * D, D, sd, &cbat))) return rc;
+    const void* d_ctx_act = bf ? t.d_ctx_act : (void*)t.d_ctx;
+    float* dst_b[8];
+    for (int i = 0; i < T; ++i) dst_b[i] = g_temb[i];
+    dst_b[T] = g_mask;
+    if (build_fused(D)) {
+        const BuildLn ln = {qnw, nullptr, cnw, nullptr, nullptr, nullptr, a.qmean, a.qrstd, a.cmean, a.crstd, d->eps};
+        if ((rc = mmae_decoder_build_bwd_ln(t.d_qn, t.d_cn, act, a.ctx_tok, d->ids_keep, d->ids_restore, d->mask_token, (const float* const*)d->task_emb, d->pos,
+                                            d->task_offsets_host, T, d->q_task, B, NC - d->G, d->G, D, n_q, &ln, bf ? t.d_ctx_act : (void*)t.d_ctx, t.part_f, st))) return rc;
+        if ((rc = fork_to(st, sd))) return rc;
+        const int nblk = mmae_decoder_build_bwd_ln_nblk((int64_t)Rq + Rc), ldp_f = (T + 5) * D;
+        float* dst_n[4] = {gb[8], gb[9], gb[6], gb[7]};
+        if ((rc = cbat.add(c, t.part_f, MMAE_F32, nblk, 4 * D, ldp_f, D, dst_n, 4, sd))) return rc;
+        if ((rc = cbat.add(c, t.part_f + 4 * D, MMAE_F32, nblk, (T + 1) * D, ldp_f, D, dst_b, T + 1, sd))) return rc;
+    } else {
     if ((rc = mmae_layernorm_bwd(t.d_qn, act, a.queries, qnw, a.qmean, a.qrstd, nullptr, t.d_queries, nullptr, MMAE_F32, t.part_q, Rq, D, st))) return rc;
     if ((rc = mmae_layernorm_bwd(t.d_cn, act, a.context, cnw, a.cmean, a.crstd, nullptr, t.d_context, nullptr, MMAE_F32, t.part_c, Rc, D, st))) return rc;
     if ((rc = mmae_decoder_build_bwd(t.d_queries, t.d_context, d->ids_keep, d->ids_restore, d->task_offsets_host, T, d->q_task, B, NC - d->G, d->G, D,
                                      n_q, t.d_ctx, t.part_b, st))) return rc;
-    const void* d_ctx_act = t.d_ctx;
-    if (bf) { if ((rc = cast_to_act(act, t.d_ctx, t.d_ctx_act, (int64_t)Rc * D, st))) return rc; d_ctx_act = t.d_ctx_act; }
+    if (bf && (rc = cast_to_act(act, t.d_ctx, t.d_ctx_act, (int64_t)Rc * D, st))) return rc;
     if ((rc = fork_to(st, sd))) return rc;
     if ((rc = cbat.add3(c, t.part_q, mmae_layernorm_bwd_nblk(Rq), D, gb[8], gb[9], nullptr, sd))) return rc;
     if ((rc = cbat.add3(c, t.part_c, mmae_layernorm_bwd_nblk(Rc), D, gb[6], gb[7], nullptr, sd))) return rc;
-    {
-        float* dst[8];
-        for (int i = 0; i < T; ++i) dst[i] = g_temb[i];
-        dst[T] = g_mask;
-        if ((rc = cbat.add(c, t.part_b, MMAE_F32, mmae_decoder_build_bwd_nblk(B), (T + 1) * D, (T + 1) * D, D, dst, T + 1, sd))) return rc;
+    if ((rc = cbat.add(c, t.part_b, MMAE_F32, mmae_decoder_build_bwd_nblk(B), (T + 1) * D, (T + 1) * D, D, dst_b, T + 1, sd))) return rc;
     }
     if (!grp_c.add(d_ctx_act, D, enc_act, d->Denc, gtail[2], gtail[3], D, d->Denc) &&
         (rc = lin_dw(c, d_ctx_act, D, enc_act, gtail[2], gtail[3], Rc, D, d->Denc, sd, &cbat))) return rc;
diff --git a/multimae_amd/csrc/rowops.hip b/multimae_amd/csrc/rowops.hip
--- a/multimae_amd/csrc/rowops.hip
+++ b/multimae_amd/csrc/rowops.hip
@@ -106,31 +106,15 @@
 #pragma unroll
         for (int i = 0; i < NV; ++i) {
             const int c = (lane + 64 * i) * 4;
-            if (c < D) {
-                const f32x4 d = d_[i], xv = xv_[i];
-#pragma unroll
-                for (int j = 0; j < 4; ++j) {
-                    xh[i][j] = (xv[j] - mu) * rs;
-                    dh[i][j] = d[j] * g[i][j];
-                    s1 += dh[i][j];
-                    s2 += dh[i][j] * xh[i][j];
-                    dg[i][j] += d[j] * xh[i][j];
-                    db[i][j] += d[j];
-                }
-            } else { xh[i] = f32x4{0.f, 0.f, 0.f, 0.f}; dh[i] = f32x4{0.f, 0.f, 0.f, 0.f}; }
+            if (c < D) ln_bwd_terms(d_[i], xv_[i], g[i], mu, rs, xh[i], dh[i], s1, s2, dg[i], db[i]);
+            else { xh[i] = f32x4{0.f, 0.f, 0.f, 0.f}; dh[i] = f32x4{0.f, 0.f, 0.f, 0.f}; }
         }
         const float c1 = wave_sum(s1) / (float)D, c2 = wave_sum(s2) / (float)D;
 #pragma unroll
         for (int i = 0; i < NV; ++i) {
             const int c = (lane + 64 * i) * 4;
             if (c < D) {
-                f32x4 o;
-#pragma unroll
-                for (int j = 0; j < 4; ++j) o[j] = rs * (dh[i][j] - c1 - xh[i][j] * c2);
-                if (dx_in) {
-#pragma unroll
-                    for (int j = 0; j < 4; ++j) o[j] += a_[i][j];
-                }
+                const f32x4 o = dx_in ? ln_bwd_dx_add(xh[i], dh[i], rs, c1, c2, a_[i]) : ln_bwd_dx(xh[i], dh[i], rs, c1, c2);
                 st4(dx_out + row * D + c, o);
                 if (dx_act) st4(dx_act + row * D + c, o);
 #pragma unroll
diff --git a/multimae_amd/csrc/tokens.hip b/multimae_amd/csrc/tokens.hip
--- a/multimae_amd/csrc/tokens.hip
+++ b/multimae_amd/csrc/tokens.hip
@@ -259,7 +259,7 @@
     }
 }
 
-template <typename YT, bool LN>
+template <typename YT, bool LN, bool SAVE = true>
 __global__ void __launch_bounds__(256) decoder_build_kernel(const float* __restrict__ ctx, const long long* __restrict__ ids_keep,
                                                             const long long* __restrict__ ids_restore, const float* __restrict__ mask_token,
                                                             const TePtrs tep, const float* __restrict__ pos, const TaskTable tt,
@@ -285,7 +285,7 @@
             const f32x4 a = ld4(base + c), t4 = te ? ld4(te + c) : f32x4{0.f, 0.f, 0.f, 0.f}, p4 = ld4(pe + c);
 #pragma unroll
             for (int k = 0; k < 4; ++k) v[k] = a[k] + (t4[k] + p4[k]);
-            st4(o + c, v);
+            if (SAVE) st4(o + c, v);
         }
         if (LN) {
             const long long row = (long long)b * n_q + j;
@@ -297,7 +297,7 @@
         float* o = context + ((long long)b * NC + r) * D;
         f32x4 v = {0.f, 0.f, 0.f, 0.f};
         if (r >= n_keep) {
-            for (int c = tl * 4; c < D; c += cstep) { v = ld4(src + c); st4(o + c, v); }
+            for (int c = tl * 4; c < D; c += cstep) { v = ld4(src + c); if (SAVE) st4(o + c, v); }
         } else {
             const int idx = (int)ids_keep[(long long)b * n_keep + r];
             const int t = task_of(tt, idx);
@@ -307,7 +307,7 @@
                 const f32x4 a = ld4(src + c), t4 = te ? ld4(te + c) : f32x4{0.f, 0.f, 0.f, 0.f}, p4 = ld4(pe + c);
 #pragma unroll
                 for (int k = 0; k < 4; ++k) v[k] = a[k] + (t4[k] + p4[k]);
-                st4(o + c, v);
+                if (SAVE) st4(o + c, v);
             }
         }
         if (LN) {
@@ -398,6 +398,167 @@
             }
         }
     }
+}
+
+constexpr int DBL_ROWS = 4 + MAX_TASKS + 1;
+template <typename DT> struct Raw4 { typedef i32x2 type; };
+template <> struct Raw4<float> { typedef f32x4 type; };
+template <typename DT> __device__ __forceinline__ f32x4 raw4_f32(const typename Raw4<DT>::type& r) { return ld4(reinterpret_cast<const DT*>(&r)); }
+template <typename DT, typename AT>
+__global__ void __launch_bounds__(256) decoder_build_bwd_ln_kernel(const DT* __restrict__ d_qn, const DT* __restrict__ d_cn, const float* __restrict__ ctx,
+                                                                   const long long* __restrict__ ids_keep, const long long* __restrict__ ids_restore,
+                                                                   const float* __restrict__ mask_token, const TePtrs tep, const float* __restrict__ pos,
+                                                                   const TaskTable tt, int q_task, int B, int n_keep, int G, int D, int n_q, int Ntot,
+                                                                   const BuildLn ln, AT* __restrict__ d_ctx, float* __restrict__ part, int part_rows) {
+    __shared__ float red[2][DBL_ROWS][256];
+    __shared__ float te_s[MAX_TASKS + 1][256];
+    const int lane = threadIdx.x & 63, w = threadIdx.x >> 6;
+    const int c = lane * 4;
+    const bool has = c < D;
+#pragma unroll
+    for (int i = 0; i <= MAX_TASKS; ++i) {
+        if ((i & 3) == w && has) {
+            const float* te = i < MAX_TASKS ? tep.p[i] : nullptr;
+            *reinterpret_cast<f32x4*>(&te_s[i][c]) = (te && i < tt.T) ? ld4(te + c) : f32x4{0.f, 0.f, 0.f, 0.f};
+        }
+    }
+    __syncthreads();
+    const int NC = n_keep + G, upb = NC + n_q;
+    const long long total = (long long)B * upb;
+    const f32x4 zero4 = {0.f, 0.f, 0.f, 0.f};
+    const f32x4 gq = has ? ld4(ln.qg + c) : zero4, gc = has ? ld4(ln.cg + c) : zero4;
+    f32x4 dgq = zero4, dbq = zero4, dgc = zero4, dbc = zero4;
+    f32x4 acc[MAX_TASKS + 1];
+#pragma unroll
+    for (int i = 0; i <= MAX_TASKS; ++i) acc[i] = zero4;
+
+    const long long step = (long long)gridDim.x * 4;
+    auto load_idx64 = [&](long long u0) -> int {
+        const long long u = u0 + lane * step;
+        if (u >= total) return 0;
+        const int b = (int)(u / upb), rr = (int)(u % upb);
+        if (rr < n_keep) return (int)ids_keep[(long long)b * n_keep + rr];
+        if (rr >= NC && q_task >= 0) return (int)ids_restore[(long long)b * Ntot + tt.off[q_task] + (rr - NC)];
+        return 0;
+    };
+    bool n_hc = false, n_hq = false, n_plain = false, n_mask = false;
+    int n_slot = -1;
+    long long n_rowc = 0;
+    typedef typename Raw4<DT>::type raw_t;
+    raw_t n_dc = {}, n_dq = {};
+    f32x4 n_a = zero4, n_p = zero4;
+    float n_muc = 0.f, n_rsc = 0.f, n_muq = 0.f, n_rsq = 0.f;
+    auto fetch = [&](long long u, int raw) {
+        const int b = (int)(u / upb), rr = (int)(u % upb);
+        n_hc = rr < NC; n_hq = false; n_plain = false; n_mask = false; n_slot = -1;
+        long long rowq = -1;
+        const float* base = nullptr; const float* pe = nullptr;
+        if (n_hc) {
+            n_rowc = (long long)b * NC + rr;
+            base = ctx + n_rowc * D;
+            n_muc = ln.cmean[n_rowc]; n_rsc = ln.crstd[n_rowc];
+            if (has) n_dc = *reinterpret_cast<const raw_t*>(d_cn + n_rowc * D + c);
+            if (rr < n_keep) {
+                const int idx = raw;
+                int t = 0, p = idx;
+#pragma unroll
+                for (int i = 1; i < MAX_TASKS; ++i) if (i < tt.T && idx >= tt.off[i]) { t = i; p = idx - tt.off[i]; }
+                pe = pos + (long long)p * D;
+                n_slot = t;
+                if (t == q_task) rowq = (long long)b * n_q + p;
+            } else n_plain = true;
+        } else if (q_task < 0 || raw >= n_keep) {
+            const int j = rr - NC;
+            rowq = (long long)b * n_q + j;
+            base = mask_token;
+            pe = pos + (long long)j * D;
+            n_slot = q_task; n_mask = true;
+        }
+        if (rowq >= 0) {
+            n_hq = true;
+            n_muq = ln.qmean[rowq]; n_rsq = ln.qrstd[rowq];
+            if (has) n_dq = *reinterpret_cast<const raw_t*>(d_qn + rowq * D + c);
+        }
+        if (has && base) {
+            n_a = ld4(base + c);
+            n_p = pe ? ld4(pe + c) : zero4;
+        }
+    };
+    auto add_slot = [&](int slot, const f32x4& o) {
+#pragma unroll
+        for (int i = 0; i < MAX_TASKS; ++i) if (i == slot) {
+#pragma unroll
+            for (int k = 0; k < 4; ++k) acc[i][k] += o[k];
+        }
+    };
+
+    long long u = (long long)blockIdx.x * 4 + w;
+    int rawv = load_idx64(u), k = 0;
+    if (u < total) fetch(u, __shfl(rawv, 0, 64));
+    for (; u < total; u += step, ++k) {
+        const bool hc = n_hc, hq = n_hq, plain = n_plain, mask = n_mask;
+        const int slot = n_slot;
+        const long long rowc = n_rowc;
+        const raw_t dc_raw = n_dc, dq_raw = n_dq;
+        const f32x4 a = n_a, p4 = n_p;
+        const float muc = n_muc, rsc = n_rsc, muq = n_muq, rsq = n_rsq;
+        if (u + step < total) {
+            if (((k + 1) & 63) == 0) rawv = load_idx64(u + step);
+            fetch(u + step, __shfl(rawv, (k + 1) & 63, 64));
+        }
+        if (!hc && !hq) continue;
+        f32x4 v = a;
+        if (!plain && has) {
+            const f32x4 t4 = *reinterpret_cast<const f32x4*>(&te_s[slot < 0 ? MAX_TASKS : slot][c]);
+#pragma unroll
+            for (int i = 0; i < 4; ++i) v[i] = a[i] + (t4[i] + p4[i]);
+        }
+        f32x4 out = zero4;
+        if (hc) {
+            f32x4 xh = zero4, dh = zero4;
+            float s1 = 0.f, s2 = 0.f;
+            if (has) ln_bwd_terms(raw4_f32<DT>(dc_raw), v, gc, muc, rsc, xh, dh, s1, s2, dgc, dbc);
+            const float c1 = wave_sum(s1) / (float)D, c2 = wave_sum(s2) / (float)D;
+            if (has) out = ln_bwd_dx(xh, dh, rsc, c1, c2);
+            add_slot(slot, out);
+        }
+        if (hq) {
+            f32x4 xh = zero4, dh = zero4, oq = zero4;
+            float s1 = 0.f, s2 = 0.f;
+            if (has) ln_bwd_terms(raw4_f32<DT>(dq_raw), v, gq, muq, rsq, xh, dh, s1, s2, dgq, dbq);
+            const float c1 = wave_sum(s1) / (float)D, c2 = wave_sum(s2) / (float)D;
+            if (has) oq = ln_bwd_dx(xh, dh, rsq, c1, c2);
+            add_slot(slot, oq);
+            if (mask) {
+#pragma unroll
+                for (int k = 0; k < 4; ++k) acc[MAX_TASKS][k] += oq[k];
+            }
+            if (hc) out = add4_rn(out, oq);
+        }
+        if (hc && has) st4(d_ctx + rowc * D + c, out);
+    }
+
+    const int nr = 4 + tt.T + 1;
+    auto put = [&](int k, const f32x4& x, bool add) {
+#pragma unroll
+        for (int j = 0; j < 4; ++j) { if (add) red[w & 1][k][c + j] += x[j]; else red[w & 1][k][c + j] = x[j]; }
+    };
+    auto put_all = [&](bool add) {
+        put(0, dgq, add); put(1, dbq, add); put(2, dgc, add); put(3, dbc, add);
+#pragma unroll
+        for (int i = 0; i < MAX_TASKS; ++i) if (i < tt.T) put(4 + i, acc[i], add);
+        put(4 + tt.T, acc[MAX_TASKS], add);
+    };
+    if (w < 2 && has) put_all(false);
+    __syncthreads();
+    if (w >= 2 && has) put_all(true);
+    __syncthreads();
+    for (int i = threadIdx.x; i < nr * D; i += 256) {
+        const int k = i / D, cc = i % D;
+        part[((long long)blockIdx.x * nr + k) * D + cc] = red[0][k][cc] + red[1][k][cc];
+    }
+    for (long long r = (long long)blockIdx.x + gridDim.x; r < part_rows; r += gridDim.x)
+        for (int i = threadIdx.x; i < nr * D; i += 256) part[r * nr * D + i] = 0.f;
 }
 
 __global__ void unpatchify_kernel(const float* __restrict__ pat, float* __restrict__ img, int C, int nh, int nw, int ph, int pw,
@@ -718,7 +879,8 @@
 int mmae_decoder_build_rows_ln(const float* ctx, const int64_t* ids_keep, const int64_t* ids_restore, const float* mask_token,
                                const float* const* task_emb_rows, const float* pos, const int32_t* task_offsets_host, int T, int q_task, int B,
                                int n_keep, int G, int D, int n_q, float* queries, float* context, const BuildLn* ln, int ln_dtype, void* stream) {
-    MMAE_REQUIRE(ctx && ids_keep && ids_restore && mask_token && task_emb_rows && pos && queries && context, "decoder_build: null pointer");
+    const bool save = queries || context || !ln;
+    MMAE_REQUIRE(ctx && ids_keep && ids_restore && mask_token && task_emb_rows && pos && (!save || (queries && context)), "decoder_build: null pointer");
     MMAE_REQUIRE(D % 4 == 0 && D <= 1024 && B > 0, "decoder_build: bad sizes");
     TaskTable tt;
     MMAE_REQUIRE(fill_tt(tt, task_offsets_host, T) == 0 && q_task >= -1 && q_task < T, "decoder_build: bad task table");
@@ -733,17 +895,46 @@
     const dim3 grid((unsigned)((total_rows + rpw - 1) / rpw));
     hipStream_t st = (hipStream_t)stream;
     const BuildLn none = {};
-#define DB_LAUNCH(YT, LN, L) hipLaunchKernelGGL((decoder_build_kernel<YT, LN>), grid, dim3(256), 0, st, ctx, (const long long*)ids_keep, \
+#define DB_LAUNCH(YT, LN, SV, L) hipLaunchKernelGGL((decoder_build_kernel<YT, LN, SV>), grid, dim3(256), 0, st, ctx, (const long long*)ids_keep, \
                        (const long long*)ids_restore, mask_token, tep, pos, tt, q_task, n_keep, G, D, n_q, tt.off[T], queries, context, total_rows, L)
+#define DB_LAUNCH_LN(YT) do { if (save) DB_LAUNCH(YT, true, true, *ln); else DB_LAUNCH(YT, true, false, *ln); } while (0)
     if (ln) {
         MMAE_REQUIRE(D <= 256 && ln->qg && ln->qb && ln->cg && ln->cb && ln->qn && ln->cn && ln->qmean && ln->qrstd && ln->cmean && ln->crstd,
                      "decoder_build: the fused LayerNorm needs D <= 256 and every output");
-        if (ln_dtype == MMAE_BF16) DB_LAUNCH(uint16_t, true, *ln);
-        else if (ln_dtype == MMAE_F16) DB_LAUNCH(h16_t, true, *ln);
-        else DB_LAUNCH(float, true, *ln);
-    } else DB_LAUNCH(float, false, none);
+        if (ln_dtype == MMAE_BF16) DB_LAUNCH_LN(uint16_t);
+        else if (ln_dtype == MMAE_F16) DB_LAUNCH_LN(h16_t);
+        else DB_LAUNCH_LN(float);
+    } else DB_LAUNCH(float, false, true, none);
+#undef DB_LAUNCH_LN
 #undef DB_LAUNCH
     return mmae_check_launch("decoder_build");
+}
+
+int mmae_decoder_build_bwd_ln_nblk(int64_t units) { const int64_t b = cdiv64(units, 4); return (int)(b < 1 ? 1 : (b > 1280 ? 1280 : b)); }
+int mmae_decoder_build_bwd_ln(const void* d_qn, const void* d_cn, int dtype, const float* ctx, const int64_t* ids_keep, const int64_t* ids_restore,
+                              const float* mask_token, const float* const* task_emb_rows, const float* pos, const int32_t* task_offsets_host, int T,
+                              int q_task, int B, int n_keep, int G, int D, int n_q, const BuildLn* ln, void* d_ctx, float* part, void* stream) {
+    MMAE_REQUIRE(d_qn && d_cn && ctx && ids_keep && ids_restore && mask_token && task_emb_rows && pos && ln && d_ctx && part, "decoder_build_bwd_ln: null pointer");
+    MMAE_REQUIRE(D % 4 == 0 && D >= 4 && D <= 256 && B > 0 && n_keep > 0 && G >= 0, "decoder_build_bwd_ln: bad sizes");
+    MMAE_REQUIRE(ln->qg && ln->cg && ln->qmean && ln->qrstd && ln->cmean && ln->crstd, "decoder_build_bwd_ln: null LayerNorm input");
+    TaskTable tt;
+    MMAE_REQUIRE(fill_tt(tt, task_offsets_host, T) == 0 && q_task >= -1 && q_task < T, "decoder_build_bwd_ln: bad task table");
+    MMAE_REQUIRE(n_q > 0 && (q_task < 0 || tt.off[q_task + 1] - tt.off[q_task] == n_q), "decoder_build_bwd_ln: n_q != tokens of the query task");
+    TePtrs tep = {};
+    for (int t = 0; t < T; ++t) {
+        MMAE_REQUIRE(((uintptr_t)task_emb_rows[t] % 16) == 0, "decoder_build_bwd_ln: unaligned task embedding");
+        tep.p[t] = task_emb_rows[t];
+    }
+    const int part_rows = mmae_decoder_build_bwd_ln_nblk((int64_t)B * (n_keep + G + n_q)), resident = mmae_cu_count() * 3;
+    const dim3 grid(part_rows < resident ? part_rows : resident);
+#define DBL_LAUNCH(DT) hipLaunchKernelGGL((decoder_build_bwd_ln_kernel<DT, DT>), grid, dim3(256), 0, (hipStream_t)stream, (const DT*)d_qn, (const DT*)d_cn, ctx, \
+                       (const long long*)ids_keep, (const long long*)ids_restore, mask_token, tep, pos, tt, q_task, B, n_keep, G, D, n_q, tt.off[T], *ln,  \
+                       (DT*)d_ctx, part, part_rows)
+    if (dtype == MMAE_BF16) DBL_LAUNCH(uint16_t);
+    else if (dtype == MMAE_F16) DBL_LAUNCH(h16_t);
+    else DBL_LAUNCH(float);
+#undef DBL_LAUNCH
+    return mmae_check_launch("decoder_build_bwd_ln");
 }
 extern "C" {
 
diff --git a/multimae_amd/ops.py b/multimae_amd/ops.py
--- a/multimae_amd/ops.py
+++ b/multimae_amd/ops.py
@@ -233,6 +233,10 @@
 
 def ln_fuse(on: Optional[bool] = None) -> bool:
     return bool(_lib.load().mmae_ln_fuse(-1 if on is None else int(bool(on))))
+
+
+def build_fuse(on: Optional[bool] = None) -> bool:
+    return bool(_lib.load().mmae_build_fuse(-1 if on is None else int(bool(on))))
 
 
 def xattn_fuse(on: Optional[bool] = None) -> bool:
```

New measurement: 8888 images/s. No clear change (-0.5%).
